# cvlab-yonsei/HVPR

Hardware: AMD Instinct MI355X
Metric: KITTI frames/sec/GPU (fwd, ~20k pts); VFE+scatter achieved HBM GB/s vs peak (higher is better)
Workload: dtype f32; 1 GPU; hvpr_car.yaml batch=1 forward-only, a1..a8 (on-GPU voxelize, pillar VFE, memory read-out + scatter, BEV backbone, head + decode, score top-k + rotated-BEV NMS); frames sharded over ranks, replicas only; global_batch=1, weights=deterministic synthetic (seed 0), BN stats randomised, cls bias -4.595

## Files before the change

### hvpr_amd/_lib.py

```python
import ctypes
import os

_HERE = os.path.dirname(os.path.abspath(__file__))
ABI_VERSION = 7
LIB_PATH = os.environ.get("HVPR_AMD_LIB", os.path.join(_HERE, "libhvpr_amd.so"))

_c = ctypes
_P = _c.c_void_p
_I = _c.c_int
_F = _c.c_float
_Z = _c.c_size_t
ALLREDUCE_FN = _c.CFUNCTYPE(_I, _P, _I, _P, _P)

SIGNATURES = {
    "hvpr_abi_version": (_I, []),
    "hvpr_status_string": (_c.c_char_p, [_I]),
    "hvpr_set_batchnorm_allreduce": (None, [_P, _P]),
    "hvpr_voxelize_workspace_bytes": (_Z, [_I, _I, _I, _I, _I]),
    "hvpr_voxelize_workspace_reset": (_I, [_P, _Z, _I, _I, _I, _I, _I, _P]),
    "hvpr_voxelize_workspace_status": (_I, [_P, _Z, _I, _I, _I, _I, _I, _P]),
    "hvpr_voxelize_f32": (_I, [_P, _I, _I, _I, _I, _P, _I, _F, _F, _F, _F, _F, _F, _I, _I, _I, _I, _I, _I,
                               _P, _P, _P, _P, _I, _P, _Z, _I, _I, _P]),
    "hvpr_pillar_vfe_fwd_f32": (_I, [_P, _P, _P, _I, _I, _P, _F, _F, _F, _F, _F, _F, _P, _P, _P, _P, _P, _P, _P, _P,
                                     _P, _P, _P, _P]),
    "hvpr_memory_bank_packed_floats": (_Z, [_I]),
    "hvpr_memory_bank_pack_f32": (_I, [_P, _I, _P, _P]),
    "hvpr_memory_readout_fwd_f32": (_I, [_P, _I, _P, _P, _P, _I, _I, _P, _P, _P]),
    "hvpr_scatter_workspace_bytes": (_Z, [_I, _I, _I]),
    "hvpr_memory_scatter_fwd_f32": (_I, [_P, _P, _P, _I, _P, _P, _P, _I, _I, _I, _I, _I, _P, _P, _P, _P, _Z, _P]),
    "hvpr_encode_fwd_f32": (_I, [_P, _I, _I, _I, _I, _P, _I, _F, _F, _F, _F, _F, _F, _I, _I, _I, _I, _I, _I, _F, _F, _F,
                                 _P, _P, _P, _P, _P, _P, _P, _P, _P, _P, _I, _I, _P, _P, _P, _P, _I, _P, _P, _P, _P, _P, _P,
                                 _P, _P, _Z, _I, _I, _I, _P]),
    "hvpr_scatter_bev_fwd_f32": (_I, [_P, _I, _P, _I, _P, _I, _P, _I, _P, _I, _I, _I, _P, _P, _P, _Z, _P]),
    "hvpr_spatial_gate_f32": (_I, [_P, _I, _I, _I, _I, _P, _F, _F, _F, _P, _P]),
    "hvpr_head_decode_f32": (_I, [_P, _I, _I, _I, _I, _I, _I, _I, _P, _P, _P, _F, _F, _F, _P, _P, _P, _P, _P]),
    "hvpr_score_topk_workspace_bytes": (_Z, [_I, _I]),
    "hvpr_score_topk_f32": (_I, [_P, _I, _I, _F, _I, _I, _P, _P, _P, _P, _Z, _P]),
    "hvpr_nms_workspace_bytes": (_Z, [_I]),
    "hvpr_nms_bev_f32": (_I, [_P, _I, _P, _P, _I, _F, _I, _I, _P, _P, _P, _Z, _P]),
    "hvpr_gather_predictions_f32": (_I, [_P, _I, _P, _P, _P, _I, _P, _P, _P, _P, _P]),
    "hvpr_boxes_pairwise_f32": (_I, [_P, _I, _P, _I, _I, _P, _P]),
    "hvpr_furthest_point_sample_f32": (_I, [_P, _I, _I, _I, _P, _P]),
    "hvpr_ball_query_f32": (_I, [_P, _P, _I, _I, _I, _F, _I, _P, _P]),
    "hvpr_three_nn_f32": (_I, [_P, _P, _I, _I, _I, _P, _P, _P]),
    "hvpr_group_points_f32": (_I, [_P, _P, _I, _I, _I, _I, _I, _P, _P]),
    "hvpr_group_points_grad_f32": (_I, [_P, _P, _I, _I, _I, _I, _I, _P, _P]),
    "hvpr_three_interpolate_f32": (_I, [_P, _P, _P, _I, _I, _I, _I, _P, _P]),
    "hvpr_three_interpolate_grad_f32": (_I, [_P, _P, _P, _I, _I, _I, _I, _P, _P]),
    "hvpr_group_rows_f32": (_I, [_P, _P, _P, _P, _I, _I, _I, _I, _I, _I, _P, _P]),
    "hvpr_max_samples_f32": (_I, [_P, _c.c_longlong, _I, _I, _P, _P, _P]),
    "hvpr_max_samples_grad_f32": (_I, [_P, _P, _c.c_longlong, _I, _I, _P, _P]),
    "hvpr_fp_rows_f32": (_I, [_P, _P, _P, _P, _I, _I, _I, _I, _I, _I, _P, _P]),
    "hvpr_spatial_gate_train_workspace_bytes": (_Z, [_I, _I, _I]),
    "hvpr_spatial_gate_train_fwd_f32": (_I, [_P, _I, _I, _I, _I, _P, _P, _P, _P, _F, _P, _P, _P, _P, _P, _P, _Z, _P]),
    "hvpr_spatial_gate_train_bwd_f32": (_I, [_P, _P, _P, _P, _P, _P, _P, _P, _I, _I, _I, _I, _P, _P, _P, _P, _P, _P, _Z, _P]),
    "hvpr_conv2d_wgrad_workspace_bytes": (_Z, [_I, _I, _I, _I, _I, _I, _I]),
    "hvpr_conv2d_wgrad_nhwc_f32": (_I, [_P, _I, _I, _I, _I, _P, _I, _I, _I, _P, _P, _Z, _P]),
    "hvpr_bn_workspace_bytes": (_Z, [_c.c_longlong, _I]),
    "hvpr_bn_stats_nhwc_f32": (_I, [_P, _c.c_longlong, _I, _F, _P, _P, _P, _P, _Z, _P]),
    "hvpr_bn_relu_fwd_nhwc_f32": (_I, [_P, _c.c_longlong, _I, _P, _P, _I, _P, _P, _P, _I, _I, _P]),
    "hvpr_bn_relu_bwd_sums_nhwc_f32": (_I, [_P, _I, _I, _P, _c.c_longlong, _I, _P, _P, _P, _P, _I, _P, _P, _P, _P, _Z, _P]),
    "hvpr_bn_relu_bwd_apply_nhwc_f32": (_I, [_P, _I, _I, _P, _c.c_longlong, _I, _P, _P, _P, _P, _I, _P, _P, _P, _P, _P, _c.c_double, _P]),
    "hvpr_memory_train_workspace_bytes": (_Z, [_I]),
    "hvpr_memory_train_fwd_f32": (_I, [_P, _c.c_longlong, _P, _I, _F, _P, _P, _P, _Z, _P]),
    "hvpr_memory_train_bwd_f32": (_I, [_P, _P, _c.c_longlong, _P, _I, _F, _P, _P, _P, _P, _P, _Z, _P]),
    "hvpr_point_pillar_topk_f32": (_I, [_P, _I, _P, _P, _I, _I, _P, _P]),
    "hvpr_scatter_add_rows_f32": (_I, [_P, _P, _c.c_longlong, _I, _I, _P, _P]),
    "hvpr_segment_sum_rows_f32": (_I, [_P, _c.c_longlong, _I, _I, _P, _P, _P, _c.c_longlong, _P, _c.c_longlong, _P]),
    "hvpr_attend_rows_fwd_f32": (_I, [_P, _I, _P, _c.c_longlong, _P, _I, _I, _P, _P, _P]),
    "hvpr_fused_adam_truewd_f32": (_I, [_P, _P, _P, _P, _c.c_longlong, _F, _F, _F, _F, _F, _I, _P, _P]),
    "hvpr_assign_targets_workspace_bytes": (_Z, [_I, _I]),
    "hvpr_assign_targets_f32": (_I, [_P, _I, _P, _I, _I, _I, _I, _F, _F, _I, _I, _I, _c.c_longlong, _P, _P, _P, _P, _P, _Z, _P]),
    "hvpr_rpn_losses_workspace_bytes": (_Z, [_I, _c.c_longlong]),
    "hvpr_rpn_losses_f32": (_I, [_P, _P, _P, _P, _P, _P, _P, _I, _c.c_longlong, _I, _I, _F, _F, _F, _P, _F, _F, _F, _F, _P, _P, _P, _P,
                                 _P, _Z, _P]),
    "hvpr_mse_loss_workspace_bytes": (_Z, []),
    "hvpr_mse_loss_f32": (_I, [_P, _P, _c.c_longlong, _I, _F, _P, _P, _P, _Z, _P]),
    "hvpr_split_bf16_f32": (_I, [_P, _c.c_longlong, _I, _P, _P]),
    "hvpr_unsplit_bf16_f32": (_I, [_P, _c.c_longlong, _I, _P, _P]),
    "hvpr_conv2d_nhwc_bf16x3": (_I, [_P, _I, _I, _I, _I, _P, _P, _I, _I, _I, _I, _P, _P, _I, _P, _I, _I, _I, _I, _I, _P]),
    "hvpr_deconv_nhwc_bf16x3": (_I, [_P, _I, _I, _I, _I, _P, _P, _I, _I, _I, _I, _P, _I, _I, _I, _P]),
    "hvpr_point_flags_f32": (_I, [_P, _I, _I, _I, _P, _F, _P, _P, _I, _I, _P, _P]),
    "hvpr_compact_workspace_bytes": (_Z, [_I]),
    "hvpr_compact_rows_f32": (_I, [_P, _I, _I, _P, _P, _I, _P, _P, _Z, _P]),
    "hvpr_frame_offsets_f32": (_I, [_P, _I, _I, _I, _P, _P]),
    "hvpr_gather_rows_f32": (_I, [_P, _I, _I, _P, _I, _P, _P]),
    "hvpr_pillar_vfe_train_workspace_bytes": (_Z, []),
    "hvpr_pillar_vfe_train_fwd_f32": (_I, [_P, _P, _P, _I, _I, _P, _P, _P, _P, _P, _P, _F, _F, _F, _F, _F, _F, _F, _P, _P, _P, _P, _P, _P, _Z, _P]),
    "hvpr_pillar_vfe_bwd_f32": (_I, [_P, _P, _P, _I, _I, _P, _P, _P, _P, _P, _P, _F, _F, _F, _F, _F, _F, _F, _P, _P, _P, _P, _P, _P, _P, _P, _Z, _P]),
    "hvpr_conv2d_wino_wgrad_workspace_bytes": (_Z, [_I, _I, _I, _I, _I]),
    "hvpr_conv2d_wino_wgrad_nhwc_f32": (_I, [_P, _I, _I, _I, _I, _P, _I, _P, _P, _Z, _P]),
    "hvpr_conv2d_wino_packed_floats": (_Z, [_I, _I]),
    "hvpr_conv2d_wino_pack_f32": (_I, [_P, _P, _I, _I, _I, _P, _P]),
    "hvpr_conv2d_wino_nhwc_f32": (_I, [_P, _I, _I, _I, _I, _P, _P, _I, _I, _P, _P, _I, _P, _I, _I, _I, _P, _P]),
    "hvpr_conv2d_wino_stats_rows": (_I, [_I, _I, _I]),
    "hvpr_conv2d_s2_dgrad_nhwc_f32": (_I, [_P, _I, _I, _I, _I, _P, _P, _I, _I, _I, _I, _P, _I, _I, _P]),
    "hvpr_bn_train_affine_f32": (_I, [_P, _P, _P, _I, _P, _P, _F, _F, _P, _P, _P, _P, _P, _P]),
    "hvpr_bn_finalize_partials_f32": (_I, [_P, _I, _I, _c.c_longlong, _F, _P, _P, _P, _P]),
    "hvpr_conv2d_nhwc_f32": (_I, [_P, _I, _I, _I, _I, _P, _P, _I, _I, _I, _I, _I, _I, _P, _P, _I, _P, _I, _I, _I, _P]),
}

_lib = None


class HvprLibraryError(RuntimeError):
    pass


def lib():
    global _lib
    if _lib is None:
        if not os.path.exists(LIB_PATH):
            raise HvprLibraryError(
                f"{LIB_PATH} is missing: build it with `python -m hvpr_amd.build` (hipcc --offload-arch=gfx950). "
                "hvpr_amd has no CPU fallback.")
        try:
            L = ctypes.CDLL(LIB_PATH)
        except OSError as e:
            raise HvprLibraryError(f"cannot load {LIB_PATH}: {e}") from e
        for name, (res, args) in SIGNATURES.items():
            fn = getattr(L, name)
            fn.restype = res
            fn.argtypes = args
        if L.hvpr_abi_version() != ABI_VERSION:
            raise HvprLibraryError(f"{LIB_PATH} has ABI version {L.hvpr_abi_version()}, these wrappers need {ABI_VERSION}: "
                                   "rebuild it with `python -m hvpr_amd.build`")
        _lib = L
    return _lib


def check(status, what):
    if status != 0:
        msg = lib().hvpr_status_string(int(status))
        raise RuntimeError(f"{what} failed: {msg.decode() if msg else status}")
```

### hvpr_amd/bev_backbone.py

```python
import collections
import contextlib
import os

import torch
import torch.nn as nn

from . import kernels
from .folding import FoldCache, bn_scale_shift


class ConvLayer(nn.Module):

    def __init__(self, in_channels, out_channels, kernel_size, stride=1, padding=0, use_norm=True, activation=False):
        super().__init__()
        self.conv = nn.Conv2d(in_channels, out_channels, kernel_size=kernel_size, stride=stride, padding=padding)
        self.norm = nn.BatchNorm2d(out_channels, eps=1e-3, momentum=0.01) if use_norm else None
        self.relu = nn.ReLU() if activation else None


class SpatialAttention(nn.Module):

    def __init__(self):
        super().__init__()
        self.spatial = ConvLayer(2, 1, 3, stride=1, padding=1, use_norm=True, activation=False)

    def gate_params(self):
        s, t = bn_scale_shift(self.spatial.norm)
        return (self.spatial.conv.weight.detach().float().reshape(18).contiguous(), float(self.spatial.conv.bias.detach()),
                float(s), float(t))


def _conv_bn_relu(cin, cout, stride=1, zero_pad=False):
    if zero_pad:
        return [nn.ZeroPad2d(1), nn.Conv2d(cin, cout, kernel_size=3, stride=stride, padding=0, bias=False),
                nn.BatchNorm2d(cout, eps=1e-3, momentum=0.01), nn.ReLU()]
    return [nn.Conv2d(cin, cout, kernel_size=3, padding=1, bias=False), nn.BatchNorm2d(cout, eps=1e-3, momentum=0.01), nn.ReLU()]


_TILE_CFG = 1
_WINO_PX_GROUPS = 1

_Level = collections.namedtuple("_Level", "index trunk scale gate sfm_steps deconv coff")
_Plan = collections.namedtuple("_Plan", "levels planes")


def _fold_pack(pack, conv, bn, **kw):
    scale, shift = bn_scale_shift(bn)
    return pack(conv.weight, scale, shift, **kw)


def _nhwc(t):
    return t.permute(0, 2, 3, 1).contiguous()


class _Fork:

    __slots__ = ("main", "sides", "used", "held", "y_event", "y_side", "eager")

    def __init__(self, sides):
        self.main, self.sides, self.used = torch.cuda.current_stream(), sides, []
        self.held = []
        self.y_event = self.y_side = None
        self.eager = not torch.cuda.is_current_stream_capturing()

    def branch(self, i, x, out):
        if not self.sides:
            return contextlib.nullcontext()
        side = self.sides[i]
        self.used.append(side)
        side.wait_stream(self.main)
        if self.y_event is not None and self.y_side is not side:
            side.wait_event(self.y_event)
        self.held.append(x)
        if self.eager:
            x.record_stream(side)
            out.record_stream(side)
        return torch.cuda.stream(side)

    def y_ready(self, i, y):
        if self.sides:
            self.y_side = self.sides[i]
            self.y_event = torch.cuda.Event()
            self.y_event.record(self.y_side)
            self.held.append(y)
            if self.eager:
                y.record_stream(self.y_side)
                if i + 1 < len(self.sides):
                    y.record_stream(self.sides[i + 1])

    def join(self):
        for side in dict.fromkeys(self.used):
            self.main.wait_stream(side)
        self.held.clear()


def _trunk(lv, x, out=None):
    for pc in lv.trunk[:-1]:
        x = kernels.conv2d_nhwc(x, pc)
    return kernels.conv2d_nhwc(x, lv.trunk[-1], out=out)


def _branch(lv, x, y, out, fork, y_out=None):
    with fork.branch(lv.index, x, out):
        y = kernels.conv2d_nhwc(y, lv.scale, out=y_out)
        fork.y_ready(lv.index, y)
        gate = kernels.spatial_gate(y, *lv.gate)
        for pc in lv.sfm_steps:
            x = kernels.conv2d_nhwc(x, pc, gate=gate, resid=x)
            fork.held.append(x)
        fork.held.append(gate)
        kernels.conv2d_nhwc(x, lv.deconv, out=out, out_coff=lv.coff)
    return y


class BaseBEVBackbone_Scale(nn.Module):

    def __init__(self, model_cfg, input_channels):
        super().__init__()
        self.model_cfg = model_cfg
        layer_nums, strides, filters = list(model_cfg.LAYER_NUMS), list(model_cfg.LAYER_STRIDES), list(model_cfg.NUM_FILTERS)
        assert len(layer_nums) == len(strides) == len(filters)
        self.sfm_layer_nums = list(model_cfg.SFM_LAYER_NUMS)
        up_strides, up_filters = list(model_cfg.UPSAMPLE_STRIDES), list(model_cfg.NUM_UPSAMPLE_FILTERS)
        assert len(up_strides) == len(up_filters) == len(layer_nums), "HIP path: one deblock per level"
        scale_filters = list(model_cfg.NUM_SCALE_FILTERS)
        assert len(scale_filters) == len(strides)
        cin = [input_channels] + filters[:-1]
        cin_s = [input_channels // 4] + scale_filters[:-1]
        self.layer_strides, self.layer_nums, self.upsample_strides = strides, layer_nums, up_strides
        self.sfmblocks_down, self.sfmblocks_up = nn.ModuleList(), nn.ModuleList()
        self.scale_layers, self.blocks, self.deblocks = nn.ModuleList(), nn.ModuleList(), nn.ModuleList()
        for i in range(len(layer_nums)):
            layers = _conv_bn_relu(cin[i], filters[i], strides[i], zero_pad=True)
            for _ in range(layer_nums[i]):
                layers += _conv_bn_relu(filters[i], filters[i])
            self.blocks.append(nn.Sequential(*layers))
            self.sfmblocks_down.append(nn.Sequential(*_conv_bn_relu(filters[i], filters[i])))
            s = up_strides[i]
            assert s >= 1 and int(s) == s, "HIP path: integer upsample strides (ConvTranspose2d with kernel == stride)"
            self.deblocks.append(nn.Sequential(
                nn.ConvTranspose2d(filters[i], up_filters[i], int(s), stride=int(s), bias=False),
                nn.BatchNorm2d(up_filters[i], eps=1e-3, momentum=0.01), nn.ReLU()))
            self.scale_layers.append(nn.Sequential(*_conv_bn_relu(cin_s[i], scale_filters[i], strides[i], zero_pad=True)))
        self.up_filters = up_filters
        self.num_bev_features = sum(up_filters)
        self.attention = SpatialAttention()
        self._fold = FoldCache()
        self._sides = None
        self.n_streams = int(os.environ.get("HVPR_BEV_STREAMS", "4"))
        self.conv_precision = os.environ.get("HVPR_CONV_PRECISION", model_cfg.get("CONV_PRECISION", "fp32"))
        assert self.conv_precision in self.PRECISIONS

    PRECISIONS = {"fp32": 0, "bf16x3": 2, "bf16x6": 3}

    def set_conv_precision(self, precision):
        assert precision in self.PRECISIONS
        self.conv_precision = precision
        self._fold.invalidate()

    def _streams(self, device):
        n = len(self.blocks)
        if self.n_streams == 1:
            return []
        if self._sides is None or len(self._sides) != n or self._sides[0].device != device:
            own = [torch.cuda.Stream(device=device) for _ in range(n if self.n_streams >= 4 else 1)]
            self._sides = [own[i % len(own)] for i in range(n)]
        return self._sides

    def train(self, mode=True):
        self._fold.invalidate()
        return super().train(mode)

    def _load_from_state_dict(self, *a, **k):
        self._fold.invalidate()
        return super()._load_from_state_dict(*a, **k)

    def _build_plan(self):
        planes = self.PRECISIONS[self.conv_precision]

        def conv_f32(conv, bn, stride=1):
            return _fold_pack(kernels.pack_conv_auto, conv, bn, stride=stride, tile_cfg=_TILE_CFG, px_groups=_WINO_PX_GROUPS)

        def conv_bf3(conv, bn, stride=1):
            return _fold_pack(kernels.pack_conv_bf3, conv, bn, stride=stride, tile_cfg=4, planes=planes)

        conv = conv_bf3 if planes else conv_f32
        gate = self.attention.gate_params()
        levels, coff = [], 0
        for i, blk in enumerate(self.blocks):
            s = self.layer_strides[i]
            trunk = [conv(blk[1], blk[2], stride=s)] + [conv(blk[4 + 3 * k], blk[5 + 3 * k]) for k in range(self.layer_nums[i])]
            sfm = conv(*self.sfmblocks_down[i][:2])
            scale = conv_f32(*self.scale_layers[i][1:3], stride=s)
            de = self.deblocks[i]
            if planes == 2 and de[0].weight.shape[0] % 64 == 0:
                deconv = _fold_pack(kernels.pack_deconv_bf3, de[0], de[1], planes=planes)
            else:
                deconv = _fold_pack(kernels.pack_deconv, de[0], de[1], tile_cfg=_TILE_CFG)
            sfm_steps = [sfm] * self.sfm_layer_nums[i]
            if planes and sfm_steps and isinstance(deconv, kernels.PackedConv):
                sfm_steps[-1] = sfm.fp32_output()
            levels.append(_Level(i, trunk, scale, gate, sfm_steps, deconv, coff))
            coff += self.up_filters[i]
        return _Plan(levels, planes)

    def _forward_train(self, data_dict):
        if not data_dict["spatial_features"].is_cuda:
            raise RuntimeError("hvpr_amd: BaseBEVBackbone_Scale's training forward needs GPU tensors (the HIP path has no CPU fallback)")
        from . import conv_train as ct

        def nhwc(t):
            return t.permute(0, 2, 3, 1).contiguous()

        def cbr(seq, t, gate=None, resid=None):
            mods, k = list(seq), 0
            while k < len(mods):
                if isinstance(mods[k], nn.ZeroPad2d):
                    k += 1
                conv, bn = mods[k], mods[k + 1]
                last = k + 3 >= len(mods)
                if last and gate is not None and resid is t and conv.stride[0] == 1 and conv.kernel_size[0] == 3:
                    t = ct.sfm_step(t, conv.weight, bn, gate)
                else:
                    z, partials = ct.conv(t, conv.weight, conv.stride[0], stats=True)
                    t = ct.bn_relu(z, bn, gate=gate if last else None, resid=resid if last else None, partials=partials)
                k += 3
            return t

        def gate(y, uses):
            sp = self.attention.spatial
            g, mean, var = ct.spatial_gate_train(y, sp.conv.weight, sp.conv.bias, sp.norm.weight, sp.norm.bias, sp.norm.eps)
            ct.update_running_repeated(sp.norm, mean, var, ct.global_count(y.numel() // y.shape[-1], y.device), uses)
            return g

        x, xp = nhwc(data_dict["spatial_features"]), nhwc(data_dict["spatial_features_point"])
        y = nhwc(data_dict["spatial_scale_features"])
        ups, ups_p = [], []
        for i in range(len(self.blocks)):
            x = cbr(self.blocks[i], x)
            xp = cbr(self.blocks[i], xp)
            y = cbr(self.scale_layers[i], y)
            xa, xpa = x, xp
            nsfm = self.sfm_layer_nums[i]
            if nsfm > 0:
                g = gate(y, 2 * nsfm)
                for _ in range(nsfm):
                    xa = cbr(self.sfmblocks_down[i], xa, gate=g, resid=xa)
                    xpa = cbr(self.sfmblocks_down[i], xpa, gate=g, resid=xpa)
            de = self.deblocks[i]
            ups.append(ct.deconv(xa, de[0].weight))
            ups_p.append(ct.deconv(xpa, de[0].weight))
        bns = [de[1] for de in self.deblocks]
        data_dict["spatial_features_2d"] = ct.bn_relu_cat(ups, bns).permute(0, 3, 1, 2)
        data_dict["spatial_features_point_2d"] = ct.bn_relu_cat(ups_p, bns).permute(0, 3, 1, 2)
        return data_dict

    def _head(self, plan, x, y, out, level, x_out={}, y_out=None):
        fork = _Fork(self._streams(y.device))
        for lv in plan.levels:
            x = _trunk(lv, x, out=x_out.get(lv.index))
            if lv.index < level:
                y = _branch(lv, x, y, out, fork, y_out=y_out if lv.index == level - 1 else None)
        fork.join()

    def forward(self, data_dict):
        if self.training:
            return self._forward_train(data_dict)
        x, y = _nhwc(data_dict["spatial_features"]), _nhwc(data_dict["spatial_scale_features"])
        plan = self._fold.get(y.device, self._build_plan)
        B, H, W, _ = x.shape
        s0, us0 = self.layer_strides[0], int(self.upsample_strides[0])
        out = torch.empty((B, ((H + 2 - 3) // s0 + 1) * us0, ((W + 2 - 3) // s0 + 1) * us0, self.num_bev_features),
                          dtype=torch.float32, device=x.device)
        if plan.planes:
            x = kernels.split_bf16(x, plan.planes)
        self._head(plan, x, y, out, len(plan.levels))
        data_dict["spatial_features_2d"] = out.permute(0, 3, 1, 2)
        return data_dict

    def forward_head(self, spatial, scale, split):
        y = _nhwc(scale)
        plan = self._fold.get(y.device, self._build_plan)
        assert not plan.planes, "the split forward runs the fp32 kernels"
        self._head(plan, _nhwc(spatial), y, split["out"], split["level"], split["x"], split["y"])

    def forward_tail(self, split):
        y, out = split["y"], split["out"]
        plan = self._fold.get(y.device, self._build_plan)
        assert not plan.planes, "the split forward runs the fp32 kernels"
        fork = _Fork([])
        for lv in plan.levels[split["level"]:]:
            y = _branch(lv, split["x"][lv.index], y, out, fork)
        fork.join()
        return out.permute(0, 3, 1, 2)

    def split_buffers(self, batch_size, H, W, device, level=None):
        n_lv = len(self.blocks)
        if level is None:
            level = n_lv - 1
        assert 1 <= level <= n_lv - 1
        h, w, hw = H, W, []
        for s in self.layer_strides:
            h, w = (h + 2 - 3) // s + 1, (w + 2 - 3) // s + 1
            hw.append((h, w))
        cy = self.scale_layers[level - 1][1].weight.shape[0]
        us0 = int(self.upsample_strides[0])
        mk = lambda *shape: torch.empty(shape, dtype=torch.float32, device=device)
        return {"level": level,
                "x": {i: mk(batch_size, hw[i][0], hw[i][1], self.blocks[i][1].weight.shape[0]) for i in range(level, n_lv)},
                "y": mk(batch_size, hw[level - 1][0], hw[level - 1][1], cy),
                "out": mk(batch_size, hw[0][0] * us0, hw[0][1] * us0, self.num_bev_features)}


__all__ = {
    "BaseBEVBackbone_Scale": BaseBEVBackbone_Scale,
}
```

### hvpr_amd/csrc/conv_wino.hip

```cpp
#include <type_traits>

#include "common.h"

namespace {

typedef float f32x16 __attribute__((ext_vector_type(16)));
constexpr int KC = 8;
constexpr int BN = 64;
constexpr int TW = 16, PW = TW + 2;
constexpr int ROWP = 20;
constexpr int W_V4 = 16 * 2 * BN;

__device__ __forceinline__ void lds_dma16(const void *sbase_uniform, unsigned voff_bytes, unsigned lds_dst_uniform) {
    unsigned keep;
    asm volatile("s_mov_b32 %0, m0\n\ts_mov_b32 m0, %3\n\ts_nop 0\n\tglobal_load_lds_dwordx4 %1, %2\n\ts_mov_b32 m0, %0"
                 : "=&s"(keep)
                 : "v"(voff_bytes), "s"(sbase_uniform), "s"(lds_dst_uniform)
                 : "memory");
}

__device__ __forceinline__ unsigned lds_addr_of(const void *p) {
    return (unsigned)(size_t)(const __attribute__((address_space(3))) void *)p;
}

struct WinoArgs {
    const float *in;
    const float *wpk;
    const float *bias;
    float *out;
    const float *gate;
    const float *resid;
    int N, H, W, Cin;
    int cout, cout_pad;
    int out_cstride, out_coff, resid_cstride;
    int relu;
    int tiles_x, tiles_y, n_ct;
    float *stats;
};

__device__ __forceinline__ float4 f4_fma(float s, float4 a, float4 b) {
    return make_float4(fmaf(s, a.x, b.x), fmaf(s, a.y, b.y), fmaf(s, a.z, b.z), fmaf(s, a.w, b.w));
}
__device__ __forceinline__ float4 f4_add(float4 a, float4 b) { return make_float4(a.x + b.x, a.y + b.y, a.z + b.z, a.w + b.w); }
__device__ __forceinline__ float4 f4_sub(float4 a, float4 b) { return make_float4(a.x - b.x, a.y - b.y, a.z - b.z, a.w - b.w); }

template <int NG, bool STATS, int NB>
__global__ void __launch_bounds__(256 * NG) __attribute__((amdgpu_waves_per_eu(2, NB == 2 ? 2 : 3))) k_wino(WinoArgs a) {
    constexpr int NT = 256 * NG;
    constexpr int TH = 8 * NG, PH = TH + 2;
    constexpr int PPAD = (PH * ROWP + 63) / 64 * 64;
    constexpr int PATCH_V4 = 2 * PPAD;
    constexpr int BNT = 32 * NB, W_V4T = 16 * 2 * BNT;
    constexpr int NLD_P = (PATCH_V4 + NT - 1) / NT, NLD_W = W_V4T / NT;
    constexpr int PATCH_PAD = NLD_P * NT;
    static_assert(W_V4T % NT == 0 && (NB == 2 || NG == 1), "whole DMA pieces");
    extern __shared__ __attribute__((aligned(16))) float4 smem[];
    float4 *const s_w = smem;
    float4 *const s_patch = smem + 2 * W_V4T;

    const int tid = threadIdx.x, lane = tid & 63, wid = tid >> 6;
    const unsigned wave_s = __builtin_amdgcn_readfirstlane((unsigned)(threadIdx.x >> 6));
    const int grp = wid >> 2, wa = wid & 3;
    const int half = lane >> 5, l31 = lane & 31;
    const int by = l31 >> 3, bx = l31 & 7;

    int p_py[NLD_P], p_px[NLD_P], p_part[NLD_P];
    bool p_live[NLD_P];
#pragma unroll
    for (int i = 0; i < NLD_P; ++i) {
        const int v = tid + i * NT;
        const int plane = v / PPAD, slot = v % PPAD;
        const int y = slot / ROWP, rem = slot % ROWP;
        const int x = 2 * (rem % 10) + rem / 10;
        p_py[i] = y; p_px[i] = x; p_part[i] = plane * 4;
        p_live[i] = plane < 2 && y < PH && x < PW;
    }
    const int r0 = wa == 0 ? 0 : (wa == 2 ? 2 : 1), r1 = wa == 2 ? 1 : (wa == 3 ? 3 : 2);
    const float sgn = wa == 1 ? 1.f : -1.f;
    const int pbase = half * PPAD + (2 * (4 * grp + by)) * ROWP + bx;
    const int p_off0 = pbase + r0 * ROWP, p_off1 = pbase + r1 * ROWP;
    const int u_off = (wa * 4 * 2 + half) * BNT + l31;
    const unsigned lds_w0 = lds_addr_of(s_w) + wave_s * 1024u;
    const unsigned lds_patch0 = lds_addr_of(s_patch) + wave_s * 1024u;

    const int n_pt = a.tiles_x * a.tiles_y * a.N;
    const int total_walk = ((n_pt + 7) / 8) * 8 * a.n_ct;
    const int n_chunks = a.Cin / KC;
    for (int it = blockIdx.x; it < total_walk; it += gridDim.x) {
    const int xcd = it & 7, j = it >> 3;
    const int ct = j % a.n_ct;
    int pt = (j / a.n_ct) * 8 + xcd;
    if (pt >= n_pt) continue;
    const int tx = pt % a.tiles_x; pt /= a.tiles_x;
    const int ty = pt % a.tiles_y;
    const int n = pt / a.tiles_y;
    const int oy0 = ty * TH, ox0 = tx * TW;
    const int iy0 = oy0 - 1, ix0 = ox0 - 1;
    const int co0 = ct * BNT;

    unsigned poff[NLD_P];
    bool pok[NLD_P];
#pragma unroll
    for (int i = 0; i < NLD_P; ++i) {
        const int iy = iy0 + p_py[i], ix = ix0 + p_px[i];
        pok[i] = p_live[i] && iy >= 0 && iy < a.H && ix >= 0 && ix < a.W;
        poff[i] = pok[i] ? (unsigned)(((iy * a.W + ix) * a.Cin + p_part[i]) * (int)sizeof(float)) : 0u;
    }
    const char *in_n = (const char *)(a.in + (size_t)n * a.H * a.W * a.Cin);
    const char *w_ct = (const char *)(a.wpk + (size_t)(NB == 2 ? ct : ct >> 1) * n_chunks * (W_V4 * 4));
    const unsigned w_half = NB == 2 ? 0u : (unsigned)(ct & 1) * 32u * 16u;

    auto stage_piece = [&](int chunk, int buf, int i) {
        if (i < NLD_P) {
            const char *pbase_g = in_n + (size_t)chunk * (KC * sizeof(float));
            if (pok[i]) lds_dma16(pbase_g, poff[i], lds_patch0 + (unsigned)(buf * PATCH_PAD + i * NT) * 16u);
        } else {
            const int j = i - NLD_P;
            const char *wbase = w_ct + (size_t)chunk * (W_V4 * 16);
            lds_dma16(wbase, NB == 2 ? (unsigned)((tid + j * NT) * 16) : (unsigned)((((tid + j * NT) >> 5) * 64 + ((tid + j * NT) & 31)) * 16) + w_half,
                      lds_w0 + (unsigned)(buf * W_V4T + j * NT) * 16u);
        }
    };
    auto stage = [&](int chunk, int buf) {
#pragma unroll
        for (int i = 0; i < NLD_P + NLD_W; ++i) stage_piece(chunk, buf, i);
    };
    const bool border = iy0 < 0 || ix0 < 0 || iy0 + PH > a.H || ix0 + PW > a.W;
    if (border) {
#pragma unroll
        for (int b = 0; b < 2; ++b)
#pragma unroll
            for (int i = 0; i < NLD_P; ++i) s_patch[b * PATCH_PAD + tid + i * NT] = make_float4(0.f, 0.f, 0.f, 0.f);
        __syncthreads();
    }
    static_assert(PH * ROWP + BNT / 4 <= PPAD, "room for the bias row behind the patch");
    if (tid < BNT / 4) s_patch[PH * ROWP + tid] = *(const float4 *)(a.bias + co0 + tid * 4);
    f32x16 acc[4][NB];
#pragma unroll
    for (int b = 0; b < 4; ++b)
#pragma unroll
        for (int nb = 0; nb < NB; ++nb)
#pragma unroll
            for (int r = 0; r < 16; ++r) acc[b][nb][r] = 0.f;

    auto chunk_step = [&](int c, auto buf_tag) {
        constexpr int BUF = decltype(buf_tag)::value;
        asm volatile("s_waitcnt vmcnt(0)" ::: "memory");
        __builtin_amdgcn_s_barrier();
        const float4 *sp = s_patch + BUF * PATCH_PAD;
        const float4 *sw = s_w + BUF * W_V4T;
        float4 d0[4], d1[4], u[4][NB];
#pragma unroll
        for (int jx = 0; jx < 4; ++jx) {
            d0[jx] = sp[p_off0 + (jx & 1) * 10 + (jx >> 1)];
            d1[jx] = sp[p_off1 + (jx & 1) * 10 + (jx >> 1)];
        }
#pragma unroll
        for (int b = 0; b < 2; ++b)
#pragma unroll
            for (int nb = 0; nb < NB; ++nb) u[b][nb] = sw[u_off + b * 2 * BNT + nb * 32];
        __builtin_amdgcn_sched_barrier(0);
        float4 t[4], v[4];
#pragma unroll
        for (int jx = 0; jx < 4; ++jx) t[jx] = f4_fma(sgn, d1[jx], d0[jx]);
        v[0] = f4_sub(t[0], t[2]); v[1] = f4_add(t[1], t[2]); v[2] = f4_sub(t[2], t[1]); v[3] = f4_sub(t[1], t[3]);
#pragma unroll
        for (int b = 0; b < 4; ++b) {
            if (b + 2 < 4) {
#pragma unroll
                for (int nb = 0; nb < NB; ++nb) u[b + 2][nb] = sw[u_off + (b + 2) * 2 * BNT + nb * 32];
            }
            __builtin_amdgcn_sched_barrier(0);
#pragma unroll
            for (int nb = 0; nb < NB; ++nb) {
                acc[b][nb] = __builtin_amdgcn_mfma_f32_32x32x2f32(u[b][nb].x, v[b].x, acc[b][nb], 0, 0, 0);
                acc[b][nb] = __builtin_amdgcn_mfma_f32_32x32x2f32(u[b][nb].y, v[b].y, acc[b][nb], 0, 0, 0);
                acc[b][nb] = __builtin_amdgcn_mfma_f32_32x32x2f32(u[b][nb].z, v[b].z, acc[b][nb], 0, 0, 0);
                acc[b][nb] = __builtin_amdgcn_mfma_f32_32x32x2f32(u[b][nb].w, v[b].w, acc[b][nb], 0, 0, 0);
                constexpr int DEAL = 4 * NB > 5 ? 5 : 4 * NB - 1, NPF = (NLD_P + NLD_W + DEAL - 1) / DEAL;
                static_assert(DEAL * NPF >= NLD_P + NLD_W, "every piece goes out");
                if (c + 1 < n_chunks && b * NB + nb < DEAL) {
                    __builtin_amdgcn_sched_barrier(0);
#pragma unroll
                    for (int i = (b * NB + nb) * NPF; i < (b * NB + nb + 1) * NPF && i < NLD_P + NLD_W; ++i) stage_piece(c + 1, BUF ^ 1, i);
                    __builtin_amdgcn_sched_barrier(0);
                }
            }
            __builtin_amdgcn_sched_barrier(0);
        }
    };
    stage(0, 0);
    for (int c = 0; c + 1 < n_chunks; c += 2) {
        chunk_step(c, std::integral_constant<int, 0>{});
        chunk_step(c + 1, std::integral_constant<int, 1>{});
    }
    if (n_chunks & 1) chunk_step(n_chunks - 1, std::integral_constant<int, 0>{});

    const int p = wa >> 1, q = wa & 1;
    const int oy = oy0 + 2 * (4 * grp + by) + p, ox = ox0 + 2 * bx + q;
    const bool live_px = oy < a.H && ox < a.W;
    const size_t pix = ((size_t)n * a.H + (live_px ? oy : 0)) * a.W + (live_px ? ox : 0);
    const float gate = a.gate && live_px ? a.gate[pix] : 0.f;
    const float *rrow = a.gate ? a.resid + pix * a.resid_cstride : nullptr;
    const float sg = p ? -1.f : 1.f;
    constexpr int NPASS = NG == 1 ? 1 : 2, NBP = NB / NPASS;
    float4 ykeep[2][4];
#pragma unroll
    for (int i = 0; i < 8; ++i) ykeep[i >> 2][i & 3] = make_float4(0.f, 0.f, 0.f, 0.f);
#pragma unroll
    for (int ps = 0; ps < NPASS; ++ps) {
        __syncthreads();
#pragma unroll
        for (int nl = 0; nl < NBP; ++nl) {
            const int nb = ps * NBP + nl;
#pragma unroll
            for (int g = 0; g < 4; ++g) {
                float4 m[4];
#pragma unroll
                for (int b = 0; b < 4; ++b) m[b] = make_float4(acc[b][nb][4 * g], acc[b][nb][4 * g + 1], acc[b][nb][4 * g + 2], acc[b][nb][4 * g + 3]);
                s_w[((((grp * 4 + wa) * 2 + 0) * NBP + nl) * 4 + g) * 64 + lane] = f4_add(f4_add(m[0], m[1]), m[2]);
                s_w[((((grp * 4 + wa) * 2 + 1) * NBP + nl) * 4 + g) * 64 + lane] = f4_sub(f4_sub(m[1], m[2]), m[3]);
            }
        }
        __syncthreads();
        if (live_px) {
#pragma unroll
            for (int nl = 0; nl < NBP; ++nl) {
                const int nb = ps * NBP + nl;
#pragma unroll
                for (int g = 0; g < 4; ++g) {
                    const int col = co0 + nb * 32 + 8 * g + 4 * half;
                    if (col >= a.cout) continue;
                    const float4 x0 = s_w[((((grp * 4 + p) * 2 + q) * NBP + nl) * 4 + g) * 64 + lane];
                    const float4 x1 = s_w[((((grp * 4 + p + 1) * 2 + q) * NBP + nl) * 4 + g) * 64 + lane];
                    const float4 x2 = s_w[((((grp * 4 + p + 2) * 2 + q) * NBP + nl) * 4 + g) * 64 + lane];
                    const float4 bias = s_patch[PH * ROWP + (col - co0) / 4];
                    float4 y = f4_add(f4_fma(sg, x2, f4_fma(sg, x1, x0)), bias);
                    if (a.relu) { y.x = fmaxf(y.x, 0.f); y.y = fmaxf(y.y, 0.f); y.z = fmaxf(y.z, 0.f); y.w = fmaxf(y.w, 0.f); }
                    if (a.gate) {
                        const float4 r = *(const float4 *)(rrow + col);
                        y.x = fmaf(gate, y.x, r.x); y.y = fmaf(gate, y.y, r.y); y.z = fmaf(gate, y.z, r.z); y.w = fmaf(gate, y.w, r.w);
                    }
                    *(float4 *)(a.out + pix * a.out_cstride + a.out_coff + col) = y;
                    if (STATS) ykeep[nl][g] = y;
                }
            }
        }
    }
    static_assert(!STATS || (NG == 1 && NB == 2), "the statistics pass is written for the 8 x 16 px x 64 channel tile");
    if (STATS) {
        __syncthreads();
#pragma unroll
        for (int nl = 0; nl < 2; ++nl)
#pragma unroll
            for (int g = 0; g < 4; ++g) s_w[((wid * 2 + nl) * 4 + g) * 64 + lane] = ykeep[nl][g];
        __syncthreads();
        {
            const int c = tid & 63, part = tid >> 6;
            const float *base = (const float *)(s_w + ((part * 2 + (c >> 5)) * 4 + ((c >> 3) & 3)) * 64 + ((c >> 2) & 1) * 32) + (c & 3);
            float sm = 0.f, sq = 0.f;
#pragma unroll 8
            for (int i = 0; i < 32; ++i) {
                const float v = base[((i + c) & 31) * 4];
                sm += v; sq = fmaf(v, v, sq);
            }
            float *s_part = (float *)(s_w + 2048);
            s_part[(part * 2 + 0) * 64 + c] = sm;
            s_part[(part * 2 + 1) * 64 + c] = sq;
        }
        __syncthreads();
        if (tid < 128) {
            const float *s_part = (const float *)(s_w + 2048);
            const int c = tid & 63, k = tid >> 6;
            const float v = (s_part[(0 * 2 + k) * 64 + c] + s_part[(1 * 2 + k) * 64 + c]) + (s_part[(2 * 2 + k) * 64 + c] + s_part[(3 * 2 + k) * 64 + c]);
            const int pt_lin = (n * a.tiles_y + ty) * a.tiles_x + tx;
            if (co0 + c < a.cout) a.stats[((size_t)pt_lin * 2 + k) * a.cout + co0 + c] = v;
        }
    }
    __syncthreads();
    }
}

__global__ void k_wino_pack(const float *__restrict__ w, const float *__restrict__ scale, int cout, int cin, int cout_pad, int adjoint,
                            float *__restrict__ out) {
    const long long id = blockIdx.x * (long long)blockDim.x + threadIdx.x;
    if (id >= (long long)cout_pad * cin) return;
    const int o = (int)(id / cin), i = (int)(id % cin);
    double g[3][3];
#pragma unroll
    for (int u = 0; u < 3; ++u)
#pragma unroll
        for (int v = 0; v < 3; ++v) {
            double x = 0.0;
            if (o < cout) x = adjoint ? (double)w[(((size_t)i * cout + o) * 3 + (2 - u)) * 3 + (2 - v)] : (double)w[(((size_t)o * cin + i) * 3 + u) * 3 + v];
            g[u][v] = (scale && o < cout) ? x * (double)scale[o] : x;
        }
    double gg[4][3];
#pragma unroll
    for (int v = 0; v < 3; ++v) {
        gg[0][v] = g[0][v];
        gg[1][v] = 0.5 * (g[0][v] + g[1][v] + g[2][v]);
        gg[2][v] = 0.5 * (g[0][v] - g[1][v] + g[2][v]);
        gg[3][v] = g[2][v];
    }
    const int ct = o / BN, co_l = o % BN, chunk = i / KC, hf = (i % KC) / 4, e = i % 4;
    float *dst = out + ((size_t)ct * (cin / KC) + chunk) * (W_V4 * 4);
#pragma unroll
    for (int r = 0; r < 4; ++r) {
        const double U[4] = {gg[r][0], 0.5 * (gg[r][0] + gg[r][1] + gg[r][2]), 0.5 * (gg[r][0] - gg[r][1] + gg[r][2]), gg[r][2]};
#pragma unroll
        for (int b = 0; b < 4; ++b) dst[(((size_t)(r * 4 + b) * 2 + hf) * BN + co_l) * 4 + e] = (float)U[b];
    }
}

template <int NG, bool STATS, int NB>
int launch(WinoArgs a, hipStream_t s) {
    constexpr int NT = 256 * NG, TH = 8 * NG, PH = TH + 2;
    constexpr int PPAD = (PH * ROWP + 63) / 64 * 64;
    constexpr int NLD_P = (2 * PPAD + NT - 1) / NT;
    constexpr int lds = (2 * (16 * 2 * 32 * NB) + 2 * NLD_P * NT) * 16;
    a.tiles_x = (a.W + TW - 1) / TW;
    a.tiles_y = (a.H + TH - 1) / TH;
    a.n_ct = a.cout_pad / (32 * NB);
    static unsigned long long lds_set = 0ull;
    if (hvpr_ensure_dyn_lds((const void *)k_wino<NG, STATS, NB>, lds, &lds_set) != 0) return -1;
    const long long tiles = (long long)a.N * a.tiles_x * a.tiles_y * a.n_ct;
    static int resident = 0;
    if (resident == 0) {
        int per_cu = 0, dev = 0, cus = 256;
        hipDeviceProp_t prop;
        if (hipGetDevice(&dev) == hipSuccess && hipGetDeviceProperties(&prop, dev) == hipSuccess) cus = prop.multiProcessorCount;
        if (hipOccupancyMaxActiveBlocksPerMultiprocessor(&per_cu, k_wino<NG, STATS, NB>, NT, lds) != hipSuccess || per_cu < 1) per_cu = 1;
        resident = per_cu * cus;
    }
    long long blocks = tiles < resident ? (tiles + 7) / 8 * 8 : resident;
    if (blocks > resident && resident >= 8) blocks = resident / 8 * 8;
    hipLaunchKernelGGL((k_wino<NG, STATS, NB>), dim3((unsigned)blocks), dim3(NT), lds, s, a);
    return 0;
}

}

extern "C" int hvpr_conv2d_wino_stats_rows(int N, int H, int W) {
    if (N < 1 || H < 1 || W < 1) return 0;
    return N * ((H + 7) / 8) * ((W + TW - 1) / TW);
}

extern "C" size_t hvpr_conv2d_wino_packed_floats(int cin, int cout) {
    if (cin < 1 || cout < 1) return 0;
    return (size_t)((cout + BN - 1) / BN * BN) * (size_t)cin * 16;
}

extern "C" int hvpr_conv2d_wino_pack_f32(const float *weight, const float *scale, int cout, int cin, int adjoint, float *packed,
                                         hvpr_stream_t stream) {
    if (!weight || !packed || cout < 1 || cin < 1) return HVPR_ERR_INVALID_ARG;
    if (cin % KC != 0) return HVPR_ERR_UNSUPPORTED;
    const int cout_pad = (cout + BN - 1) / BN * BN;
    const long long n = (long long)cout_pad * cin;
    hipLaunchKernelGGL(k_wino_pack, dim3(hvpr_cdiv(n, 256)), dim3(256), 0, (hipStream_t)stream, weight, scale, cout, cin, cout_pad,
                       adjoint ? 1 : 0, packed);
    HVPR_CHECK_LAUNCH();
    return HVPR_OK;
}

extern "C" int hvpr_conv2d_wino_nhwc_f32(const float *in, int N, int H, int W, int Cin, const float *w_packed, const float *bias,
                                         int cout, int relu, const float *gate, const float *resid, int resid_cstride, float *out,
                                         int out_cstride, int out_coff, int px_groups, float *bn_partials, hvpr_stream_t stream) {
    if (!in || !w_packed || !bias || !out || N < 1 || H < 1 || W < 1 || Cin < 8 || cout < 1) return HVPR_ERR_INVALID_ARG;
    if ((gate == nullptr) != (resid == nullptr)) return HVPR_ERR_INVALID_ARG;
    if (Cin % KC != 0) return HVPR_ERR_UNSUPPORTED;
    if (cout % 4 != 0 || out_cstride % 4 != 0 || out_coff % 4 != 0 || (resid && resid_cstride % 4 != 0)) return HVPR_ERR_UNSUPPORTED;
    if ((long long)H * W * Cin * 4 >= (1ll << 31)) return HVPR_ERR_UNSUPPORTED;
    WinoArgs a;
    a.in = in; a.wpk = w_packed; a.bias = bias; a.out = out; a.gate = gate; a.resid = resid;
    a.N = N; a.H = H; a.W = W; a.Cin = Cin;
    a.cout = cout; a.cout_pad = (cout + BN - 1) / BN * BN;
    a.out_cstride = out_cstride; a.out_coff = out_coff; a.resid_cstride = resid_cstride;
    a.relu = relu;
    a.stats = bn_partials;
    if (bn_partials && (px_groups != 1 || relu || gate)) return HVPR_ERR_UNSUPPORTED;
    int rc;
    if (px_groups == 1) rc = bn_partials ? launch<1, true, 2>(a, (hipStream_t)stream) : launch<1, false, 2>(a, (hipStream_t)stream);
    else if (px_groups == 2) rc = launch<2, false, 2>(a, (hipStream_t)stream);
    else if (px_groups == 4) rc = launch<1, false, 1>(a, (hipStream_t)stream);
    else return HVPR_ERR_INVALID_ARG;
    if (rc != 0) return HVPR_ERR_LAUNCH;
    HVPR_CHECK_LAUNCH();
    return HVPR_OK;
}
```

### hvpr_amd/csrc/internal.h

```cpp
#pragma once
#include "common.h"

#define HVPR_INTERNAL __attribute__((visibility("hidden")))

constexpr int kScanThreads = 256;
constexpr int kScanItems = 2;
constexpr int kScanTile = kScanThreads * kScanItems;
constexpr int kIdle = 0x7fffffff;

struct VoxWs {
    int *cell_first;
    int *cell_count;
    int *cell_vid;
    int *pt_cell;
    int4 *vox_rec;
    int *arena;
    float4 *arena_pt;
    int4 *arena_rec;
    int *arena_total;
    float *vfe_aux;
    int *frame_base;
    unsigned long long *tile_state;
    int *ticket;
    unsigned long long *cell_pack;
    int *sync;
};

static inline VoxWs hvpr_vox_carve(void *ws, int batch, int n, long long ncell, size_t *bytes = nullptr) {
    hvpr_carver c(ws);
    VoxWs w;
    w.cell_first = c.take<int>((size_t)batch * ncell);
    w.cell_count = c.take<int>((size_t)batch * ncell);
    w.cell_vid = c.take<int>((size_t)batch * ncell);
    w.pt_cell = c.take<int>(n);
    w.vox_rec = c.take<int4>(n);
    w.arena = c.take<int>(n);
    w.arena_pt = c.take<float4>(n);
    w.arena_rec = c.take<int4>(n);
    w.arena_total = c.take<int>(1);
    w.vfe_aux = c.take<float>(128);
    w.frame_base = c.take<int>(batch + 1);
    w.tile_state = c.take<unsigned long long>(hvpr_cdiv(n > 0 ? n : 1, kScanTile));
    w.ticket = c.take<int>(1);
    w.cell_pack = c.take<unsigned long long>((size_t)batch * ncell);
    w.sync = c.take<int>(8 + 64);
    if (bytes) *bytes = c.off;
    return w;
}

static inline size_t hvpr_vox_ws_bytes(int batch, int n, long long ncell) {
    size_t bytes = 0;
    hvpr_vox_carve(nullptr, batch, n, ncell, &bytes);
    return bytes;
}

struct ClearJob {
    int *cell_first;
    int *cell_count;
    const int *cell_vid;
    const int *frame_base;
    const int *voxel_offsets;
    int batch, nx, ny, max_voxels, capacity;
    float *spatial;
    float *spatial_scale;
    long long cell_lo, cell_hi;
    unsigned char *state;
};

__device__ __forceinline__ void hvpr_canvas_clear(const ClearJob &c, int blk, int nblk) {
    constexpr int V = 32, VS = 8;
    typedef float f32x4 __attribute__((ext_vector_type(4)));
    const int lane = threadIdx.x & 63;
    const long long wave = ((long long)blk * blockDim.x + threadIdx.x) >> 6, n_waves = ((long long)nblk * blockDim.x) >> 6;
    const f32x4 zero = {0.f, 0.f, 0.f, 0.f};
    for (long long c0 = c.cell_lo + wave * 64; c0 < c.cell_hi; c0 += n_waves * 64) {
        const long long cell = c0 + lane;
        bool emitted = false, stale = c.state == nullptr;
        if (cell < c.cell_hi) {
            if (c.state) stale = c.state[cell] != 0;
            if (c.cell_first[cell] != kIdle) {
                c.cell_first[cell] = kIdle;
                c.cell_count[cell] = 0;
                const int b = (int)(cell / ((long long)c.nx * c.ny));
                const int local = c.cell_vid[cell] - c.frame_base[b];
                emitted = local < c.max_voxels && c.voxel_offsets[b] + local < c.capacity;
            }
            if (c.state && stale != emitted) c.state[cell] = emitted ? 1 : 0;
        }
        const unsigned long long skip = __ballot(emitted || !stale);
        if (c.state && skip == ~0ull) continue;
        f32x4 *const main = reinterpret_cast<f32x4 *>(c.spatial) + c0 * V;
        f32x4 *const side = reinterpret_cast<f32x4 *>(c.spatial_scale) + c0 * VS;
        const int cells = (int)min(64ll, c.cell_hi - c0);
#pragma unroll 8
        for (int i = lane; i < cells * V; i += 64)
            if (!((skip >> (i / V)) & 1ull)) __builtin_nontemporal_store(zero, main + i);
#pragma unroll 8
        for (int i = lane; i < cells * VS; i += 64)
            if (!((skip >> (i / VS)) & 1ull)) __builtin_nontemporal_store(zero, side + i);
    }
}

typedef float hvpr_f32x16 __attribute__((ext_vector_type(16)));
__device__ __forceinline__ void hvpr_vfe_padded_slot(const float (&aw)[2][8], const float (&b0h)[8], float *z1) {
    const int lane = threadIdx.x & 63, h = lane >> 5, slot = lane & 31;
#pragma unroll
    for (int mb = 0; mb < 2; ++mb) {
        hvpr_f32x16 acc = {0.f, 0.f, 0.f, 0.f, 0.f, 0.f, 0.f, 0.f, 0.f, 0.f, 0.f, 0.f, 0.f, 0.f, 0.f, 0.f};
#pragma unroll
        for (int t = 0; t < 8; ++t) acc = __builtin_amdgcn_mfma_f32_32x32x2f32(aw[mb][t], fmaxf(0.f + b0h[t], 0.f), acc, 0, 0, 0);
        if (slot == 0) {
#pragma unroll
            for (int g = 0; g < 4; ++g) *(float4 *)&z1[32 * mb + 8 * g + 4 * h] = make_float4(acc[4 * g], acc[4 * g + 1], acc[4 * g + 2], acc[4 * g + 3]);
        }
    }
}

struct VoxelizeArgs {
    const float *points;
    int n_points, point_stride, xyz_col, n_feat;
    const int32_t *frame_offsets;
    int batch;
    float lo_x, lo_y, lo_z, vs_x, vs_y, vs_z;
    int nx, ny, nz, max_points, max_voxels, cap_mode;
};

struct VfeWeights {
    float vs_x, vs_y, vs_z, off_x, off_y, off_z;
    const float *w0, *b0, *w1, *b1, *ws0, *bs0, *ws1, *bs1;
};

struct WarmSmall { const float *p[8]; int n[8]; };
HVPR_INTERNAL int hvpr_i_voxel_index(const VoxelizeArgs &a, const VoxWs &w, int32_t *voxel_offsets, bool for_encode,
                                     hipStream_t s, const float *vfe_w1 = nullptr, const float *vfe_b0 = nullptr,
                                     const void *warm0 = nullptr, size_t warm0_bytes = 0, const void *warm1 = nullptr, size_t warm1_bytes = 0,
                                     const WarmSmall *warm_small = nullptr, int index_mode = 0);
HVPR_INTERNAL int hvpr_i_vfe_gather(const VoxelizeArgs &a, const VoxWs &w, const int32_t *voxel_offsets, int capacity,
                                    const VfeWeights &v, float *voxels, int32_t *coords, int32_t *num_points,
                                    float *pillar_features, float *scale_features, float *pillar_mask, float *spatial,
                                    int spatial_channels, float *spatial_scale, unsigned char *canvas_state, hipStream_t s);
HVPR_INTERNAL int hvpr_i_readout(const float *f, int M, const int32_t *m_device, const float *bank, const float *bank_packed, int n_items, int k,
                                 float *out, int32_t *topk_idx, const int32_t *coords, int batch, int nx, int ny,
                                 int *cell_map, float *canvas, int canvas_channels, int canvas_offset, hipStream_t s);
```

### hvpr_amd/detector.py

```python
import os

import numpy as np
import torch
import torch.nn as nn

from . import anchor_head, bev_backbone, iou3d_nms_utils, kernels, map_to_bev, pointnet2, vfe
from .voxel_generator import VoxelGenerator

backbones_3d_all = pointnet2.__all__
REGISTRY = {
    "backbone_3d": backbones_3d_all,
    "vfe": vfe.__all__,
    "map_to_bev": map_to_bev.__all__,
    "backbone_2d": bev_backbone.__all__,
    "dense_head": anchor_head.__all__,
}


def class_agnostic_nms(box_scores, box_preds, nms_config, score_thresh=None):
    n = box_scores.shape[0]
    dev = box_scores.device
    if n == 0:
        return torch.zeros((0,), dtype=torch.long, device=dev), box_scores[:0]
    pre = min(int(nms_config.NMS_PRE_MAXSIZE), n)
    ws = kernels.PostWorkspace(1, n, pre, dev)
    order, _, cnt = kernels.score_topk(box_scores.float().reshape(1, n).contiguous(), score_thresh, pre, ws, want_scores=False)
    keep, kc = kernels.nms_bev(box_preds.float().contiguous(), order[0].contiguous(), cnt, pre, float(nms_config.NMS_THRESH),
                               int(nms_config.NMS_POST_MAXSIZE), ws.nms)
    selected = keep[: int(kc.item())].long()
    return selected, box_scores[selected]


def multi_classes_nms(cls_scores, box_preds, nms_config, score_thresh=None):
    pred_scores, pred_labels, pred_boxes = [], [], []
    for k in range(cls_scores.shape[1]):
        col = cls_scores[:, k].contiguous()
        selected, sc = class_agnostic_nms(col, box_preds, nms_config, score_thresh=score_thresh)
        pred_scores.append(sc)
        pred_labels.append(torch.full((selected.shape[0],), k, dtype=torch.long, device=col.device))
        pred_boxes.append(box_preds[selected])
    return torch.cat(pred_scores, dim=0), torch.cat(pred_labels, dim=0), torch.cat(pred_boxes, dim=0)


class Detector3DTemplate(nn.Module):

    def __init__(self, model_cfg, num_class, dataset):
        super().__init__()
        self.model_cfg = model_cfg
        self.num_class = num_class
        self.dataset = dataset
        self.class_names = dataset.class_names
        self.register_buffer("global_step", torch.LongTensor(1).zero_())
        self.module_topology = ["backbone_3d", "vfe", "map_to_bev_module", "pfe", "backbone_2d", "dense_head",
                                "point_head", "roi_head"]
        self._post_ws = None

    @property
    def mode(self):
        return "TRAIN" if self.training else "TEST"

    def update_global_step(self):
        self.global_step += 1

    def build_networks(self):
        info = {
            "module_list": [],
            "num_rawpoint_features": self.dataset.point_feature_encoder.num_point_features,
            "num_point_features": self.dataset.point_feature_encoder.num_point_features,
            "grid_size": self.dataset.grid_size,
            "point_cloud_range": self.dataset.point_cloud_range,
            "voxel_size": self.dataset.voxel_size,
        }
        for name in self.module_topology:
            module, info = getattr(self, "build_%s" % name)(model_info_dict=info)
            self.add_module(name, module)
        return info["module_list"]

    def build_backbone_3d(self, model_info_dict):
        cfg = self.model_cfg.get("BACKBONE_3D", None)
        if cfg is None or cfg.NAME not in backbones_3d_all:
            return None, model_info_dict
        m = backbones_3d_all[cfg.NAME](model_cfg=cfg, input_channels=model_info_dict["num_point_features"],
                                       grid_size=model_info_dict["grid_size"], voxel_size=model_info_dict["voxel_size"],
                                       point_cloud_range=model_info_dict["point_cloud_range"])
        model_info_dict["module_list"].append(m)
        model_info_dict["num_point_features"] = m.num_point_features
        return m, model_info_dict

    def build_vfe(self, model_info_dict):
        cfg = self.model_cfg.get("VFE", None)
        if cfg is None:
            return None, model_info_dict
        m = vfe.__all__[cfg.NAME](model_cfg=cfg, num_point_features=model_info_dict["num_rawpoint_features"],
                                  point_cloud_range=model_info_dict["point_cloud_range"], voxel_size=model_info_dict["voxel_size"])
        model_info_dict["num_point_features"] = m.get_output_feature_dim()
        model_info_dict["module_list"].append(m)
        return m, model_info_dict

    def build_map_to_bev_module(self, model_info_dict):
        cfg = self.model_cfg.get("MAP_TO_BEV", None)
        if cfg is None:
            return None, model_info_dict
        m = map_to_bev.__all__[cfg.NAME](model_cfg=cfg, grid_size=model_info_dict["grid_size"])
        model_info_dict["module_list"].append(m)
        model_info_dict["num_bev_features"] = m.num_bev_features
        return m, model_info_dict

    def build_backbone_2d(self, model_info_dict):
        cfg = self.model_cfg.get("BACKBONE_2D", None)
        if cfg is None:
            return None, model_info_dict
        m = bev_backbone.__all__[cfg.NAME](model_cfg=cfg, input_channels=model_info_dict["num_bev_features"])
        model_info_dict["module_list"].append(m)
        model_info_dict["num_bev_features"] = m.num_bev_features
        return m, model_info_dict

    def build_dense_head(self, model_info_dict):
        cfg = self.model_cfg.get("DENSE_HEAD", None)
        if cfg is None:
            return None, model_info_dict
        m = anchor_head.__all__[cfg.NAME](
            model_cfg=cfg, input_channels=model_info_dict["num_bev_features"],
            num_class=self.num_class if not cfg.CLASS_AGNOSTIC else 1, class_names=self.class_names,
            grid_size=model_info_dict["grid_size"], point_cloud_range=model_info_dict["point_cloud_range"],
            predict_boxes_when_training=self.model_cfg.get("ROI_HEAD", False))
        model_info_dict["module_list"].append(m)
        return m, model_info_dict

    def _absent(self, key, model_info_dict):
        assert self.model_cfg.get(key, None) is None, f"{key} is outside the hvpr hot path"
        return None, model_info_dict

    def build_pfe(self, model_info_dict):
        return self._absent("PFE", model_info_dict)

    def build_point_head(self, model_info_dict):
        return self._absent("POINT_HEAD", model_info_dict)

    def build_roi_head(self, model_info_dict):
        return self._absent("ROI_HEAD", model_info_dict)

    def forward(self, **kwargs):
        raise NotImplementedError

    def post_processing(self, batch_dict, sync=True):
        cfg = self.model_cfg.POST_PROCESSING
        ncfg = cfg.NMS_CONFIG
        if ncfg.MULTI_CLASSES_NMS:
            return self._post_processing_multi_class(batch_dict)
        B = batch_dict["batch_size"]
        boxes_all = batch_dict["batch_box_preds"]
        assert boxes_all.dim() == 3 and boxes_all.shape[0] == B
        cls_all = batch_dict["batch_cls_preds"]
        assert cls_all.shape[2] in (1, self.num_class)
        if "batch_max_scores" in batch_dict:
            scores, labels = batch_dict["batch_max_scores"], batch_dict["batch_max_labels"]
        else:
            c = cls_all if batch_dict["cls_preds_normalized"] else torch.sigmoid(cls_all)
            scores, lab = torch.max(c, dim=-1)
            labels = (lab + 1).to(torch.int32)
        A = scores.shape[1]
        pre, post = min(int(ncfg.NMS_PRE_MAXSIZE), A), int(ncfg.NMS_POST_MAXSIZE)
        dev = scores.device
        if self._post_ws is None or (self._post_ws.batch, self._post_ws.n_scores, self._post_ws.pre_max) != (B, A, pre) \
                or self._post_ws.topk.device != dev:
            self._post_ws = kernels.PostWorkspace(B, A, pre, dev)
        order, _, counts = kernels.score_topk(scores.contiguous(), cfg.SCORE_THRESH, pre, self._post_ws, want_scores=False)
        pred_dicts, recall_dict = [], {}
        for b in range(B):
            keep, kc = kernels.nms_bev(boxes_all[b], order[b], counts[b:b + 1], pre, float(ncfg.NMS_THRESH), post,
                                       self._post_ws.nms)
            if labels.dtype == torch.int32 and not cfg.OUTPUT_RAW_SCORE and boxes_all[b].is_contiguous():
                pb, ps, pl, sel = kernels.gather_predictions(boxes_all[b], scores[b].contiguous(), labels[b].contiguous(), keep)
                rec = {"pred_boxes": pb, "pred_labels": pl, "pred_scores": ps, "selected": sel, "pred_count": kc}
            else:
                sel = keep.long()
                rec = {"pred_boxes": boxes_all[b].index_select(0, sel), "pred_labels": labels[b].index_select(0, sel).long(),
                       "pred_scores": (cls_all[b].max(dim=-1)[0] if cfg.OUTPUT_RAW_SCORE else scores[b]).index_select(0, sel),
                       "selected": sel, "pred_count": kc}
            if sync:
                n = int(kc.item())
                rec = {k: (v[:n] if k != "pred_count" else v) for k, v in rec.items()}
                recall_dict = self.generate_recall_record(rec["pred_boxes"], recall_dict, b, batch_dict, cfg.RECALL_THRESH_LIST)
            pred_dicts.append(rec)
        return pred_dicts, recall_dict, batch_dict

    def _post_processing_multi_class(self, batch_dict):
        cfg = self.model_cfg.POST_PROCESSING
        pred_dicts, recall_dict = [], {}
        for b in range(batch_dict["batch_size"]):
            cls = batch_dict["batch_cls_preds"][b]
            cls = cls if batch_dict["cls_preds_normalized"] else torch.sigmoid(cls)
            boxes = batch_dict["batch_box_preds"][b]
            mapping = torch.arange(1, cls.shape[1] + 1, device=cls.device)
            sc, lab, bx = multi_classes_nms(cls.float(), boxes, cfg.NMS_CONFIG, score_thresh=cfg.SCORE_THRESH)
            rec = {"pred_boxes": bx, "pred_scores": sc, "pred_labels": mapping[lab]}
            recall_dict = self.generate_recall_record(bx, recall_dict, b, batch_dict, cfg.RECALL_THRESH_LIST)
            pred_dicts.append(rec)
        return pred_dicts, recall_dict, batch_dict

    @staticmethod
    def generate_recall_record(box_preds, recall_dict, batch_index, data_dict=None, thresh_list=None):
        if "gt_boxes" not in data_dict:
            return recall_dict
        gt = data_dict["gt_boxes"][batch_index]
        if len(recall_dict) == 0:
            recall_dict = {"gt": 0}
            for t in thresh_list:
                recall_dict["roi_%s" % str(t)] = 0
                recall_dict["rcnn_%s" % str(t)] = 0
        row_is_zero = (gt.sum(dim=1) == 0).tolist()
        k = len(row_is_zero) - 1
        while k > 0 and row_is_zero[k]:
            k -= 1
        gt = gt[:k + 1]
        if gt.shape[0] > 0:
            if box_preds.shape[0] > 0:
                best = iou3d_nms_utils.boxes_iou3d_gpu(box_preds[:, 0:7], gt[:, 0:7]).max(dim=0)[0]
                thr = torch.tensor([float(t) for t in thresh_list], dtype=best.dtype).to(best.device, non_blocking=True)
                recalled = (best.unsqueeze(0) > thr.unsqueeze(1)).sum(dim=1).tolist()
                for t, n in zip(thresh_list, recalled):
                    recall_dict["rcnn_%s" % str(t)] += int(n)
            recall_dict["gt"] += gt.shape[0]
        return recall_dict

    def load_params_from_file(self, filename, logger=None, to_cpu=False):
        ckpt = torch.load(filename, map_location=torch.device("cpu") if to_cpu else None)
        disk = ckpt["model_state"]
        state = self.state_dict()
        update = {k: v for k, v in disk.items() if k in state and state[k].shape == v.shape}
        state.update(update)
        self.load_state_dict(state)
        from . import conv_train
        conv_train.weights_changed()
        if logger is not None:
            for k in state:
                if k not in update:
                    logger.info("Not updated weight %s: %s" % (k, str(state[k].shape)))
            logger.info("==> Done (loaded %d/%d)" % (len(update), len(state)))
        return len(update), len(state)


    def load_params_with_optimizer(self, filename, to_cpu=False, optimizer=None, logger=None):
        if not os.path.isfile(filename):
            raise FileNotFoundError(filename)
        ckpt = torch.load(filename, map_location=torch.device("cpu") if to_cpu else None)
        self.load_state_dict(ckpt["model_state"])
        if optimizer is not None:
            ost = ckpt.get("optimizer_state")
            if ost is None:
                stem, ext = os.path.splitext(filename)
                side = "%s_optim%s" % (stem, ext)
                if os.path.exists(side):
                    ost = torch.load(side, map_location=torch.device("cpu") if to_cpu else None)["optimizer_state"]
            if ost is not None:
                optimizer.load_state_dict(ost)
        if logger is not None:
            logger.info("==> Resumed from %s (epoch %s, it %s, version %s)" % (filename, ckpt.get("epoch", -1), ckpt.get("it", 0.0),
                                                                              ckpt.get("version", "none")))
        return ckpt.get("it", 0.0), ckpt.get("epoch", -1)


class _VoxelizingDetector(Detector3DTemplate):

    def __init__(self, model_cfg, num_class, dataset):
        super().__init__(model_cfg=model_cfg, num_class=num_class, dataset=dataset)
        self._voxgen = {}

    def _voxel_cfg(self):
        for p in self.dataset.dataset_cfg.DATA_PROCESSOR:
            if p.NAME == "transform_points_to_voxels":
                return p
        raise KeyError("transform_points_to_voxels")

    def _voxel_generator(self, device):
        mode = "train" if self.training else "test"
        key = (mode, torch.device(device))
        if key not in self._voxgen:
            vc = self._voxel_cfg()
            self._voxgen[key] = VoxelGenerator(vc.VOXEL_SIZE, self.dataset.point_cloud_range, vc.MAX_POINTS_PER_VOXEL,
                                               vc.MAX_NUMBER_OF_VOXELS[mode], device=device)
        return self._voxgen[key]

    @staticmethod
    def _frame_offsets(batch_dict):
        offs = batch_dict.get("point_frame_offsets")
        if offs is None:
            pts, B = batch_dict["points"], batch_dict["batch_size"]
            if pts.is_cuda and pts.dtype == torch.float32 and pts.is_contiguous():
                offs = kernels.frame_offsets(pts, B)
            else:
                offs = torch.searchsorted(pts[:, 0].contiguous(), torch.arange(B + 1, device=pts.device, dtype=pts.dtype)).to(torch.int32)
        return offs

    def voxelize_on_device(self, batch_dict):
        pts = batch_dict["points"]
        B = batch_dict["batch_size"]
        offs = self._frame_offsets(batch_dict)
        v, c, n, vo = self._voxel_generator(pts.device).generate_batch(pts, offs, B, xyz_col=1, n_feat=pts.shape[1] - 1)
        batch_dict["voxels"], batch_dict["voxel_coords"], batch_dict["voxel_num_points"] = v, c, n
        batch_dict["voxel_offsets"] = vo
        batch_dict["voxel_count_device"] = vo[B:B + 1]
        return batch_dict


class MixAnchor_Memory(_VoxelizingDetector):

    def __init__(self, model_cfg, num_class, dataset):
        super().__init__(model_cfg=model_cfg, num_class=num_class, dataset=dataset)
        self.module_list = self.build_networks()
        self.export_voxels = bool(model_cfg.get("EXPORT_VOXELS", False))
        self.index_mode = int(model_cfg.get("ENCODE_INDEX_MODE", 1))

    def get_training_loss(self):
        rpn, rpn_point, mem, tb_dict, items = self.dense_head.get_loss()
        loss = rpn + rpn_point + mem
        tb_dict = {"loss_rpn": rpn.detach(), **tb_dict}
        return loss, tb_dict, {"items": items}

    def _can_fuse_encode(self, batch_dict):
        if self.training or "voxels" in batch_dict:
            return False
        v, m = getattr(self, "vfe", None), getattr(self, "map_to_bev_module", None)
        if not isinstance(v, vfe.PillarVFE_Scale) or not isinstance(m, map_to_bev.PointPillarScatter_Agg_Memory_1_scale):
            return False
        pts = batch_dict["points"]
        return (pts.is_cuda and pts.dim() == 2 and pts.shape[1] == 5 and v.num_filters == [32, 64] and
                v.num_scale_features == [16, 32] and tuple(m.memory.weight.shape[1:]) == (64,) and m.nz == 1 and
                int(self._voxel_cfg().MAX_POINTS_PER_VOXEL) <= 32 and m.memory.weight.shape[0] <= 2048 and m.k <= 32)

    def encode_fused(self, batch_dict):
        pts, B = batch_dict["points"].contiguous(), batch_dict["batch_size"]
        vg = self._voxel_generator(pts.device)
        m = self.map_to_bev_module
        r = kernels.encode_fwd(pts, self._frame_offsets(batch_dict), B, vg.point_cloud_range, vg.voxel_size, vg.grid_size,
                               vg.max_num_points, vg.max_voxels, vg._workspace(B, pts.shape[0]),
                               self.vfe._fold.get(pts.device, self.vfe._build_folded), self.vfe.offsets,
                               m.memory.packed_bank(), m.k, xyz_col=1, cap_mode=vg.cap_mode, want_voxels=self.export_voxels,
                               want_mask=self.export_voxels, out=batch_dict.get("_out_spatial"), state=batch_dict.get("_canvas_state"),
                               index_mode=self.index_mode)
        vo = r["voxel_offsets"]
        batch_dict.update(voxels=r["voxels"], voxel_coords=r["coords"], voxel_num_points=r["num_points"], voxel_offsets=vo,
                          voxel_count_device=vo[B:B + 1], pillar_features=r["pillar_features"],
                          pillar_scale_features=r["pillar_scale_features"], pillar_mask=r["pillar_mask"],
                          spatial_features=r["spatial"], spatial_scale_features=r["spatial_scale"])
        return batch_dict

    def persistent_canvases(self, example_batch):
        if not self._can_fuse_encode(example_batch):
            return {}
        m = self.map_to_bev_module
        canv, state = kernels.canvas_buffers(example_batch["batch_size"], m.nx, m.ny, example_batch["points"].device)
        return {"_out_spatial": canv, "_canvas_state": state}

    def stage_encode(self, batch_dict):
        if self._can_fuse_encode(batch_dict):
            return self.encode_fused(batch_dict)
        if "voxels" not in batch_dict:
            batch_dict = self.voxelize_on_device(batch_dict)
        return self.map_to_bev_module(self.vfe(batch_dict))

    def stage_dense(self, batch_dict):
        return self.dense_head(self.backbone_2d(batch_dict))

    def stage_dense_a(self, batch_dict, split):
        self.backbone_2d.forward_head(batch_dict["spatial_features"], batch_dict["spatial_scale_features"], split)

    def stage_dense_b(self, batch_dict, split):
        return self.dense_head({**batch_dict, "spatial_features_2d": self.backbone_2d.forward_tail(split)})

    def prefetch_point_indices(self, batch_dict):
        pn = getattr(self, "backbone_3d", None)
        if pn is None or not hasattr(pn, "index_plan") or "points" not in batch_dict or not batch_dict["points"].is_cuda:
            return batch_dict
        if getattr(self, "_pn2_stream", None) is None:
            self._pn2_stream = torch.cuda.Stream()
        s = self._pn2_stream
        s.wait_stream(torch.cuda.current_stream())
        with torch.cuda.stream(s):
            plan = pn.index_plan(batch_dict["points"], batch_dict["batch_size"])
            ready = torch.cuda.Event()
            ready.record(s)
        batch_dict["points"].record_stream(s)
        batch_dict["_pn2_plan"] = (plan, ready)
        return batch_dict

    def forward(self, batch_dict, sync=True):
        fused = self._can_fuse_encode(batch_dict)
        if fused:
            batch_dict = self.encode_fused(batch_dict)
        elif "voxels" not in batch_dict:
            batch_dict = self.voxelize_on_device(batch_dict)
        if self.training:
            for m in self.module_list:
                batch_dict = m(batch_dict)
            loss, tb_dict, disp_dict = self.get_training_loss()
            return {"loss": loss}, tb_dict, disp_dict
        for m in self.module_list:
            if m is getattr(self, "backbone_3d", None) or (fused and (m is self.vfe or m is self.map_to_bev_module)):
                continue
            batch_dict = m(batch_dict)
        out = self.post_processing(batch_dict, sync=sync)
        if fused and sync and self.index_mode == 1:
            self._voxel_generator(batch_dict["points"].device)._ws.status()
        return out


class _CapturedState:

    def __init__(self, model):
        self.slots = []
        for m in model.modules():
            if hasattr(m, "_fold") and hasattr(m._fold, "value"):
                self.slots.append((m._fold, "value"))
            if hasattr(m, "_packed"):
                self.slots.append((m, "_packed"))
        self.slots.append((model, "_post_ws"))
        for vg in getattr(model, "_voxgen", {}).values():
            self.slots.append((vg, "_ws"))
        self.keep = [getattr(o, a) for o, a in self.slots]

    def check(self):
        for (o, a), was in zip(self.slots, self.keep):
            if getattr(o, a) is not was:
                raise RuntimeError(f"hvpr_amd: {type(o).__name__}.{a} was rebuilt after this hipGraph was captured (train()/eval(), "
                                   "load_state_dict, set_conv_precision or a workspace re-allocation): capture a new graph")


def _check_voxelizer_status(model):
    for vg in getattr(model, "_voxgen", {}).values():
        if vg._ws is not None:
            vg._ws.status()


class GraphedForward:

    def __init__(self, model, example_batch, warmup=3):
        assert not model.training
        self.model = model
        self.static_in = {k: (v.clone() if torch.is_tensor(v) else v) for k, v in example_batch.items()}
        if hasattr(model, "persistent_canvases"):
            self.static_in.update(model.persistent_canvases(example_batch))
        side = torch.cuda.Stream()
        side.wait_stream(torch.cuda.current_stream())
        with torch.cuda.stream(side), torch.no_grad():
            for _ in range(warmup):
                model(dict(self.static_in), sync=False)
        torch.cuda.current_stream().wait_stream(side)
        torch.cuda.synchronize()
        self.graph = torch.cuda.CUDAGraph()
        with torch.cuda.graph(self.graph), torch.no_grad():
            self.static_out = model(dict(self.static_in), sync=False)
        self.captured = _CapturedState(model)

    def __call__(self, batch):
        self.captured.check()
        for k, v in batch.items():
            if torch.is_tensor(v):
                self.static_in[k].copy_(v, non_blocking=True)
        self.graph.replay()
        return self.static_out

    def check_status(self):
        _check_voxelizer_status(self.model)


class PipelinedForward:

    _HEAD_KEYS = ("batch_cls_preds", "batch_box_preds", "batch_max_scores", "batch_max_labels")

    def __init__(self, model, example_batch, warmup=2, depth=None):
        assert not model.training and hasattr(model, "stage_encode")
        if depth is None:
            fp32 = getattr(model.backbone_2d, "conv_precision", "fp32") == "fp32" and hasattr(model.backbone_2d, "split_buffers")
            depth = 4 if fp32 else 3
        assert depth in (3, 4)
        self.model, self.step, self.depth = model, 0, depth
        self.B = example_batch["batch_size"]
        self.inp = [{k: (v.clone() if torch.is_tensor(v) else v) for k, v in example_batch.items()} for _ in range(2)]
        self.canvas, self.head, self.aux, self.split = [None, None], [None, None], [None, None], [None, None]
        self.enc, self.f2d = [None, None], [None, None]
        self.own = [model.persistent_canvases(example_batch) if hasattr(model, "persistent_canvases") else {} for _ in range(2)]
        side = torch.cuda.Stream()
        side.wait_stream(torch.cuda.current_stream())
        with torch.cuda.stream(side), torch.no_grad():
            for p in range(2):
                for _ in range(warmup):
                    bd = model.stage_encode({**self.inp[p], **self.own[p]})
                    self.canvas[p] = (bd["spatial_features"], bd["spatial_scale_features"])
                    if depth == 4:
                        if self.split[p] is None:
                            sp = bd["spatial_features"]
                            self.split[p] = model.backbone_2d.split_buffers(self.B, sp.shape[2], sp.shape[3], sp.device)
                        model.stage_dense_a(bd, self.split[p])
                        bd = model.stage_dense_b(bd, self.split[p])
                    else:
                        bd = model.stage_dense(bd)
                    self.head[p] = tuple(bd[k] for k in self._HEAD_KEYS)
                    model.post_processing(bd, sync=False)
        torch.cuda.current_stream().wait_stream(side)
        torch.cuda.synchronize()
        self.s_enc, self.s_post, self.s_b = torch.cuda.Stream(), torch.cuda.Stream(), torch.cuda.Stream()
        self.graphs, self.out = [torch.cuda.CUDAGraph(), torch.cuda.CUDAGraph()], [None, None]
        pool = None
        for p in range(2):
            q = 1 - p
            post_lane = p if depth == 3 else q
            with torch.cuda.graph(self.graphs[p], pool=pool), torch.no_grad():
                main = torch.cuda.current_stream()
                self.s_enc.wait_stream(main)
                self.s_post.wait_stream(main)
                with torch.cuda.stream(self.s_post):
                    self.out[p] = model.post_processing(self._post_dict(post_lane), sync=False)[0]
                with torch.cuda.stream(self.s_enc):
                    bd = model.stage_encode({**self.inp[p], "_out_spatial": self.canvas[p], **self.own[p]})
                    self.aux[p] = bd["voxel_offsets"]
                    self.enc[p] = {k: bd[k] for k in ("voxel_coords", "voxel_num_points", "voxel_offsets", "pillar_features",
                                                      "pillar_scale_features") if bd.get(k) is not None}
                dense_in = {"batch_size": self.B, "spatial_features": self.canvas[q][0], "spatial_scale_features": self.canvas[q][1]}
                if depth == 3:
                    self.f2d[q] = model.stage_dense({**dense_in, "_out_head": self.head[q]})["spatial_features_2d"]
                else:
                    self.s_b.wait_stream(main)
                    with torch.cuda.stream(self.s_b):
                        model.stage_dense_b({"batch_size": self.B, "_out_head": self.head[p]}, self.split[p])
                    model.stage_dense_a(dense_in, self.split[q])
                    main.wait_stream(self.s_b)
                main.wait_stream(self.s_enc)
                main.wait_stream(self.s_post)
            pool = self.graphs[p].pool()
        self.captured = _CapturedState(model)

    def _post_dict(self, p):
        d = dict(zip(self._HEAD_KEYS, self.head[p]))
        d.update(batch_size=self.B, cls_preds_normalized=False)
        return d

    def __call__(self, batch):
        self.captured.check()
        p = self.step & 1
        for k, v in batch.items():
            if torch.is_tensor(v):
                self.inp[p][k].copy_(v, non_blocking=True)
        self.graphs[p].replay()
        self.step += 1
        return self.out[p] if self.step >= self.depth else None

    def inspect(self, batch):
        for _ in range(self.depth):
            out = self(batch)
        torch.cuda.synchronize()
        self.check_status()
        p = (self.step - 1) & 1
        q = 1 - p
        d = {k: v.clone() for k, v in self.enc[p].items()}
        d["spatial_features"], d["spatial_scale_features"] = self.canvas[p][0].clone(), self.canvas[p][1].clone()
        if self.depth == 4:
            d["spatial_features_2d"] = self.split[p]["out"].permute(0, 3, 1, 2).clone()
            head_now, head_post = self.head[p], self.head[q]
        else:
            d["spatial_features_2d"] = self.f2d[q].clone()
            head_now, head_post = self.head[q], self.head[p]
        d.update({k: v.clone() for k, v in zip(self._HEAD_KEYS, head_now)})
        d["post_input"] = {k: v.clone() for k, v in zip(self._HEAD_KEYS, head_post)}
        d["post"] = [{k: (v.clone() if torch.is_tensor(v) else v) for k, v in rec.items()} for rec in out]
        return d

    def check_status(self):
        _check_voxelizer_status(self.model)

    def flush(self):
        for _ in range(self.depth - 1):
            p = self.step & 1
            self.graphs[p].replay()
            self.step += 1
            if self.step >= self.depth:
                yield self.out[p]


class PointPillar(_VoxelizingDetector):

    def __init__(self, model_cfg, num_class, dataset):
        super().__init__(model_cfg=model_cfg, num_class=num_class, dataset=dataset)
        self.module_list = self.build_networks()

    def forward(self, batch_dict, sync=True):
        if self.training:
            raise NotImplementedError("hvpr_amd: plain PointPillar has no training path (the reference's own detectors/pointpillar.py:24-32 unpacks "
                                      "two values from a get_loss that returns five, anchor_head_template.py:291); train MixAnchor_Memory")
        if "voxels" not in batch_dict:
            batch_dict = self.voxelize_on_device(batch_dict)
        for m in self.module_list:
            batch_dict = m(batch_dict)
        return self.post_processing(batch_dict, sync=sync)


__all__ = {
    "Detector3DTemplate": Detector3DTemplate,
    "PointPillar": PointPillar,
    "MixAnchor_Memory": MixAnchor_Memory,
}


def build_detector(model_cfg, num_class, dataset):
    return __all__[model_cfg.NAME](model_cfg=model_cfg, num_class=num_class, dataset=dataset)


def build_network(model_cfg, num_class, dataset):
    return build_detector(model_cfg=model_cfg, num_class=num_class, dataset=dataset)


def load_data_to_gpu(batch_dict):
    for k, v in batch_dict.items():
        if not isinstance(v, np.ndarray) or k in ("frame_id", "metadata", "calib", "image_shape"):
            continue
        batch_dict[k] = torch.from_numpy(v).float().cuda()


class SyntheticDataset:

    class _Encoder:
        def __init__(self, n):
            self.num_point_features = n

    def __init__(self, cfg, training=False):
        from .voxel_generator import grid_size_of
        self.dataset_cfg = cfg.DATA_CONFIG
        self.class_names = list(cfg.CLASS_NAMES)
        self.training = training
        self.point_cloud_range = np.array(self.dataset_cfg.POINT_CLOUD_RANGE, dtype=np.float32)
        self.point_feature_encoder = self._Encoder(len(self.dataset_cfg.POINT_FEATURE_ENCODING.used_feature_list))
        vc = [p for p in self.dataset_cfg.DATA_PROCESSOR if p.NAME == "transform_points_to_voxels"][0]
        self.voxel_size = vc.VOXEL_SIZE
        self.grid_size = grid_size_of(self.point_cloud_range, self.voxel_size)
```

### hvpr_amd/kernels.py

```python
import os

import torch

from ._lib import check, lib


def _stream():
    return torch.cuda.current_stream().cuda_stream


def _ptr(t, dtype=None, name="tensor"):
    if t is None:
        return None
    if not t.is_cuda:
        raise RuntimeError(f"hvpr_amd: {name} must live on the GPU (the HIP path has no CPU fallback)")
    if dtype is not None and t.dtype != dtype:
        raise TypeError(f"hvpr_amd: {name} must be {dtype}, got {t.dtype}")
    if not t.is_contiguous():
        raise ValueError(f"hvpr_amd: {name} must be contiguous")
    return t.data_ptr()


class VoxelizeWorkspace:

    def __init__(self, batch, n_points, grid, device):
        self.key = (int(batch), int(n_points), tuple(int(g) for g in grid), torch.device(device))
        nx, ny, nz = self.key[2]
        nbytes = lib().hvpr_voxelize_workspace_bytes(batch, n_points, nx, ny, nz)
        self.buf = torch.empty(nbytes, dtype=torch.uint8, device=device)
        self.reset()

    def reset(self):
        batch, n_points, (nx, ny, nz), _ = self.key
        check(lib().hvpr_voxelize_workspace_reset(self.buf.data_ptr(), self.buf.numel(), batch, n_points, nx, ny, nz,
                                                  _stream()), "hvpr_voxelize_workspace_reset")

    def status(self):
        batch, n_points, (nx, ny, nz), _ = self.key
        check(lib().hvpr_voxelize_workspace_status(self.buf.data_ptr(), self.buf.numel(), batch, n_points, nx, ny, nz,
                                                   _stream()), "hvpr_voxelize_workspace_status")


def voxelize(points, frame_offsets, batch, point_cloud_range, voxel_size, grid, max_points, max_voxels, workspace,
             xyz_col=0, n_feat=None, cap_mode=0, capacity=None):
    n, stride = points.shape
    n_feat = stride - xyz_col if n_feat is None else n_feat
    if capacity is None:
        capacity = min(n, batch * max_voxels)
    dev = points.device
    voxels = torch.empty((capacity, max_points, n_feat), dtype=torch.float32, device=dev)
    coords = torch.empty((capacity, 4), dtype=torch.int32, device=dev)
    num = torch.empty((capacity,), dtype=torch.int32, device=dev)
    offs = torch.empty((batch + 1,), dtype=torch.int32, device=dev)
    nx, ny, nz = [int(g) for g in grid]
    lo = [float(torch.tensor(v, dtype=torch.float32)) for v in point_cloud_range[:3]]
    vs = [float(torch.tensor(v, dtype=torch.float32)) for v in voxel_size]
    if workspace.key[0] < batch or workspace.key[1] < n:
        raise ValueError("voxelize workspace too small for this call")
    check(lib().hvpr_voxelize_f32(_ptr(points, torch.float32, "points"), n, stride, xyz_col, n_feat,
                                  _ptr(frame_offsets, torch.int32, "frame_offsets"), batch, lo[0], lo[1], lo[2],
                                  vs[0], vs[1], vs[2], nx, ny, nz, int(max_points), int(max_voxels), int(cap_mode),
                                  voxels.data_ptr(), coords.data_ptr(), num.data_ptr(), offs.data_ptr(), capacity,
                                  workspace.buf.data_ptr(), workspace.buf.numel(), workspace.key[0], workspace.key[1],
                                  _stream()), "hvpr_voxelize_f32")
    return voxels, coords, num, offs


def pillar_vfe_fwd(voxels, num_points, coords, folded, voxel_size, offsets, m_device=None, want_mask=True):
    M, P, C = voxels.shape
    if C != 4:
        raise ValueError("hvpr_pillar_vfe_fwd_f32 is built for 4 raw point features")
    dev = voxels.device
    pf = torch.empty((M, 64), dtype=torch.float32, device=dev)
    sf = torch.empty((M, 32), dtype=torch.float32, device=dev)
    mask = torch.empty((M, P, 1), dtype=torch.float32, device=dev) if want_mask else None
    check(lib().hvpr_pillar_vfe_fwd_f32(
        _ptr(voxels, torch.float32, "voxels"), _ptr(num_points, torch.int32, "voxel_num_points"),
        _ptr(coords, torch.int32, "voxel_coords"), M, P, _ptr(m_device, torch.int32, "m_device"),
        float(voxel_size[0]), float(voxel_size[1]), float(voxel_size[2]), float(offsets[0]), float(offsets[1]),
        float(offsets[2]), _ptr(folded["w0"], torch.float32), _ptr(folded["b0"], torch.float32),
        _ptr(folded["w1"], torch.float32), _ptr(folded["b1"], torch.float32), _ptr(folded["ws0"], torch.float32),
        _ptr(folded["bs0"], torch.float32), _ptr(folded["ws1"], torch.float32), _ptr(folded["bs1"], torch.float32),
        pf.data_ptr(), sf.data_ptr(), _ptr(mask), _stream()), "hvpr_pillar_vfe_fwd_f32")
    return pf, sf, mask


class PackedBank:

    def __init__(self, weight):
        w = weight.detach().float().contiguous()
        if w.dim() != 2 or w.shape[1] != 64:
            raise ValueError("PackedBank: (n_items, 64) memory bank expected")
        self.n_items = int(w.shape[0])
        self.shape = w.shape
        self.rows = w
        self.data = torch.empty(lib().hvpr_memory_bank_packed_floats(self.n_items), dtype=torch.float32, device=w.device)
        check(lib().hvpr_memory_bank_pack_f32(_ptr(w, torch.float32, "memory.weight"), self.n_items, self.data.data_ptr(), _stream()),
              "hvpr_memory_bank_pack_f32")


def _bank_args(bank):
    if not isinstance(bank, PackedBank):
        _ptr(bank, torch.float32, "memory.weight")
        bank = PackedBank(bank)
    return bank.rows.data_ptr(), bank.data.data_ptr(), bank.n_items


def memory_readout_fwd(f, bank, k, m_device=None, want_idx=False):
    M, C = f.shape
    out = torch.empty((M, C), dtype=torch.float32, device=f.device)
    idx = torch.empty((M, k), dtype=torch.int32, device=f.device) if want_idx else None
    check(lib().hvpr_memory_readout_fwd_f32(_ptr(f, torch.float32, "pillar_features"), M,
                                            _ptr(m_device, torch.int32, "m_device"), *_bank_args(bank), int(k),
                                            out.data_ptr(), _ptr(idx), _stream()), "hvpr_memory_readout_fwd_f32")
    return (out, idx) if want_idx else out


_SEG_CHUNK = 32


def edges_by_destination(dst, n_dst):
    dst = dst.reshape(-1).to(torch.int64)
    dev = dst.device
    E = dst.numel()
    n_max = E // _SEG_CHUNK + min(n_dst, E) + 1
    if E == 0:
        z = torch.zeros(1, dtype=torch.int32, device=dev)
        return torch.zeros(0, dtype=torch.int32, device=dev), z.expand(n_max + 1).contiguous(), z.expand(n_dst + 1).contiguous()
    order = torch.argsort(dst, stable=True)
    sdst = dst[order].contiguous()
    rowptr = torch.searchsorted(sdst, torch.arange(n_dst + 1, dtype=torch.int64, device=dev))
    end_live = rowptr[n_dst:]
    pos = torch.arange(E, dtype=torch.int64, device=dev)
    live = (sdst >= 0) & (sdst < n_dst)
    first = rowptr[sdst.clamp(0, n_dst - 1)]
    head = live & (((pos - first) % _SEG_CHUNK) == 0)
    csum = torch.cumsum(head.to(torch.int64), 0)
    cid, total = csum - 1, csum[-1:]
    chunk_ptr = end_live.expand(n_max + 1).clone()
    chunk_ptr.scatter_(0, torch.where(head, cid, torch.full_like(cid, n_max)), torch.where(head, pos, end_live.expand(E)))
    dest_ptr = torch.where(rowptr < end_live, cid[rowptr.clamp(max=E - 1)], total.expand(n_dst + 1))
    return order.to(torch.int32), chunk_ptr.to(torch.int32), dest_ptr.to(torch.int32)


def segment_sum_rows(src, src_off, C, edge_row, edge_w, chunk_ptr, dest_ptr, n_dst):
    n_chunks = chunk_ptr.numel() - 1
    part = torch.empty((n_chunks, C), dtype=torch.float32, device=src.device)
    check(lib().hvpr_segment_sum_rows_f32(_ptr(src, torch.float32, "src"), src.shape[-1], int(src_off), int(C), _ptr(edge_row, torch.int32, "edge_row"),
                                          _ptr(edge_w, torch.float32, "edge_w"), _ptr(chunk_ptr, torch.int32, "chunk_ptr"), int(n_chunks),
                                          part.data_ptr(), int(C), _stream()), "hvpr_segment_sum_rows_f32")
    dst = torch.empty((n_dst, C), dtype=torch.float32, device=src.device)
    check(lib().hvpr_segment_sum_rows_f32(part.data_ptr(), int(C), 0, int(C), None, None, _ptr(dest_ptr, torch.int32, "dest_ptr"), int(n_dst),
                                          dst.data_ptr(), int(C), _stream()), "hvpr_segment_sum_rows_f32")
    return dst


def attend_rows(q, rows, idx=None, k=None):
    if idx is not None:
        if idx.dim() != 2 or (k is not None and int(k) != idx.shape[1]):
            raise ValueError("hvpr_amd: attend_rows needs idx of shape (M, k)")
        k = idx.shape[1]
    elif k is None:
        raise ValueError("hvpr_amd: attend_rows without idx needs k")
    M, C = q.shape
    if rows.dim() != 2 or rows.shape[1] != C or (idx is not None and idx.shape[0] != M):
        raise ValueError("hvpr_amd: attend_rows needs q (M, C), rows (N, C) and idx (M, k)")
    qp, rp, ip = _ptr(q, torch.float32, "q"), _ptr(rows, torch.float32, "rows"), _ptr(idx, torch.int32, "idx")
    out = torch.empty((M, C), dtype=torch.float32, device=q.device)
    w = torch.empty((M, int(k)), dtype=torch.float32, device=q.device)
    check(lib().hvpr_attend_rows_fwd_f32(qp, M, rp, rows.shape[0], ip, int(k), C, out.data_ptr(), w.data_ptr(), _stream()),
          "hvpr_attend_rows_fwd_f32")
    return out, w


def scatter_workspace(batch, nx, ny, device):
    n = lib().hvpr_scatter_workspace_bytes(batch, nx, ny) // 4
    return torch.full((n,), -1, dtype=torch.int32, device=device)


def scatter_bev_fwd(pillar, memory, scale, coords, batch, nx, ny, workspace, m_device=None):
    M, cp = pillar.shape
    cm = 0 if memory is None else memory.shape[1]
    cs = 0 if scale is None else scale.shape[1]
    dev = pillar.device
    spatial = torch.empty((batch, ny, nx, cp + cm), dtype=torch.float32, device=dev)
    spatial_scale = torch.empty((batch, ny, nx, cs), dtype=torch.float32, device=dev) if cs else None
    check(lib().hvpr_scatter_bev_fwd_f32(_ptr(pillar, torch.float32, "pillar_features"), cp, _ptr(memory, torch.float32),
                                         cm, _ptr(scale, torch.float32), cs, _ptr(coords, torch.int32, "voxel_coords"),
                                         M, _ptr(m_device, torch.int32), batch, nx, ny, spatial.data_ptr(),
                                         _ptr(spatial_scale), workspace.data_ptr(), workspace.numel() * 4, _stream()),
          "hvpr_scatter_bev_fwd_f32")
    spatial = spatial.permute(0, 3, 1, 2)
    if spatial_scale is not None:
        spatial_scale = spatial_scale.permute(0, 3, 1, 2)
    return spatial, spatial_scale


class PackedConvBf3:

    def __init__(self, w, bias, cin, cout, cout_pad, stride, relu, tile_cfg, planes, up=None, out_split=True):
        self.w, self.bias, self.cin, self.cout, self.cout_pad = w, bias, cin, cout, cout_pad
        self.stride, self.relu, self.tile_cfg, self.planes, self.up, self.out_split = stride, relu, tile_cfg, planes, up, out_split

    def fp32_output(self):
        return PackedConvBf3(self.w, self.bias, self.cin, self.cout, self.cout_pad, self.stride, self.relu, self.tile_cfg, self.planes,
                             out_split=False)


def _planes_of(x, planes):
    out, r = [], x
    for _ in range(planes):
        h = r.to(torch.bfloat16)
        out.append(h)
        r = r - h.float()
    return out


def pack_conv_bf3(weight, scale=None, shift=None, stride=1, relu=True, tile_cfg=0, planes=2):
    cout, cin, kh, kw = weight.shape
    assert kh == kw == 3 and cin % 16 == 0 and cout % 4 == 0 and planes in (2, 3)
    w = weight.detach().float()
    if scale is not None:
        w = w * scale.view(-1, 1, 1, 1)
    cout_pad = (cout + 63) // 64 * 64
    wp = torch.zeros((9, cin // 8, planes, cout_pad, 8), dtype=torch.bfloat16, device=w.device)
    for k, part in enumerate(_planes_of(w, planes)):
        wp[:, :, k, :cout, :] = part.permute(2, 3, 1, 0).reshape(9, cin // 8, 8, cout).permute(0, 1, 3, 2)
    b = torch.zeros((cout_pad,), dtype=torch.float32, device=w.device)
    if shift is not None:
        b[:cout] = shift.detach().float()
    return PackedConvBf3(wp.contiguous(), b, cin, cout, cout_pad, stride, relu, tile_cfg, planes)


def pack_deconv_bf3(weight, scale, shift, relu=True, planes=2):
    cin, cout, s, s2 = weight.shape
    assert s == s2 and cin % 64 == 0 and cout % 4 == 0 and planes in (2, 3)
    w = weight.detach().float() * scale.view(1, -1, 1, 1)
    cols = s * s * cout
    cout_pad = (cols + 63) // 64 * 64
    g = w.permute(0, 2, 3, 1).reshape(cin, cols)
    wp = torch.zeros((1, cin // 8, planes, cout_pad, 8), dtype=torch.bfloat16, device=w.device)
    for k, part in enumerate(_planes_of(g, planes)):
        wp[0, :, k, :cols, :] = part.reshape(cin // 8, 8, cols).permute(0, 2, 1)
    b = torch.zeros((cout_pad,), dtype=torch.float32, device=w.device)
    b[:cols] = shift.detach().float().repeat(s * s)
    return PackedConvBf3(wp.contiguous(), b, cin, cout, cout_pad, 1, relu, 1, planes, up=s)


def deconv_nhwc_bf3(xs, pc, out, out_coff=0):
    N, H, W, groups, planes, _ = xs.shape
    assert groups * 8 == pc.cin and planes == pc.planes and xs.is_contiguous()
    assert out.shape[:3] == (N, H * pc.up, W * pc.up) and out.is_contiguous() and out.dtype == torch.float32
    check(lib().hvpr_deconv_nhwc_bf16x3(xs.data_ptr(), N, H, W, pc.cin, pc.w.data_ptr(), pc.bias.data_ptr(), pc.cout, pc.cout_pad,
                                        pc.up, 1 if pc.relu else 0, out.data_ptr(), out.shape[-1], out_coff, planes, _stream()),
          "hvpr_deconv_nhwc_bf16x3")
    return out


def split_bf16(x, planes=2):
    assert x.is_contiguous() and x.shape[-1] % 8 == 0 and x.dtype == torch.float32
    out = torch.empty((*x.shape[:-1], x.shape[-1] // 8, planes, 8), dtype=torch.bfloat16, device=x.device)
    check(lib().hvpr_split_bf16_f32(_ptr(x, torch.float32, "activations"), x.numel(), planes, out.data_ptr(), _stream()),
          "hvpr_split_bf16_f32")
    return out


def unsplit_bf16(xs):
    assert xs.is_contiguous() and xs.dtype == torch.bfloat16 and xs.shape[-1] == 8
    planes = xs.shape[-2]
    out = torch.empty((*xs.shape[:-3], xs.shape[-3] * 8), dtype=torch.float32, device=xs.device)
    check(lib().hvpr_unsplit_bf16_f32(xs.data_ptr(), out.numel(), planes, out.data_ptr(), _stream()), "hvpr_unsplit_bf16_f32")
    return out


def conv2d_nhwc_bf3(xs, pc, out_split=True, gate=None, resid=None):
    N, H, W, groups, planes, _ = xs.shape
    cin = groups * 8
    assert cin == pc.cin and planes == pc.planes and xs.is_contiguous()
    OH, OW = (H + 2 - 3) // pc.stride + 1, (W + 2 - 3) // pc.stride + 1
    if out_split:
        assert pc.cout % 8 == 0
        out = torch.empty((N, OH, OW, pc.cout // 8, planes, 8), dtype=torch.bfloat16, device=xs.device)
    else:
        out = torch.empty((N, OH, OW, pc.cout), dtype=torch.float32, device=xs.device)
    check(lib().hvpr_conv2d_nhwc_bf16x3(xs.data_ptr(), N, H, W, cin, pc.w.data_ptr(), pc.bias.data_ptr(), pc.stride, pc.cout,
                                        pc.cout_pad, 1 if pc.relu else 0, _ptr(gate, torch.float32, "gate"),
                                        None if resid is None else resid.data_ptr(), 0 if resid is None else resid.shape[3] * 8,
                                        out.data_ptr(), 1 if out_split else 0, pc.cout, 0, pc.tile_cfg, planes, _stream()),
          "hvpr_conv2d_nhwc_bf16x3")
    return out


def memory_scatter_fwd(pillar, scale, coords, bank, k, batch, nx, ny, workspace, m_device=None, out=None):
    M = pillar.shape[0]
    dev = pillar.device
    mem = torch.empty((M, 64), dtype=torch.float32, device=dev)
    if out is not None:
        spatial, spatial_scale = (o.permute(0, 2, 3, 1) for o in out)
        if spatial.shape != (batch, ny, nx, 128) or spatial_scale.shape != (batch, ny, nx, 32) or not spatial.is_contiguous() \
                or not spatial_scale.is_contiguous():
            raise ValueError("memory_scatter_fwd: `out` canvases do not match this call")
    else:
        spatial = torch.empty((batch, ny, nx, 128), dtype=torch.float32, device=dev)
        spatial_scale = torch.empty((batch, ny, nx, 32), dtype=torch.float32, device=dev)
    if pillar.shape[1] != 64 or scale.shape[1] != 32 or bank.shape[1] != 64:
        raise ValueError("memory_scatter_fwd is specialised for 64 pillar / 64 memory / 32 scale channels")
    check(lib().hvpr_memory_scatter_fwd_f32(_ptr(pillar, torch.float32, "pillar_features"), _ptr(scale, torch.float32, "scale"),
                                            _ptr(coords, torch.int32, "voxel_coords"), M, _ptr(m_device, torch.int32),
                                            *_bank_args(bank), int(k), batch, nx, ny,
                                            mem.data_ptr(), spatial.data_ptr(), spatial_scale.data_ptr(), workspace.data_ptr(),
                                            workspace.numel() * 4, _stream()), "hvpr_memory_scatter_fwd_f32")
    return mem, spatial.permute(0, 3, 1, 2), spatial_scale.permute(0, 3, 1, 2)


def frame_offsets(points, batch):
    offs = torch.empty((batch + 1,), dtype=torch.int32, device=points.device)
    check(lib().hvpr_frame_offsets_f32(_ptr(points, torch.float32, "points"), points.shape[0], points.shape[1], int(batch),
                                       offs.data_ptr(), _stream()), "hvpr_frame_offsets_f32")
    return offs


def encode_fwd(points, frame_offsets, batch, point_cloud_range, voxel_size, grid, max_points, max_voxels, workspace, folded,
               offsets, bank, k, xyz_col=0, cap_mode=0, capacity=None, want_voxels=True, want_mask=True, out=None, state=None,
               index_mode=0):
    n, stride = points.shape
    n_feat = stride - xyz_col
    if capacity is None:
        capacity = min(n, batch * max_voxels)
    dev = points.device
    nx, ny, nz = [int(g) for g in grid]
    voxels = torch.empty((capacity, max_points, n_feat), dtype=torch.float32, device=dev) if want_voxels else None
    coords = torch.empty((capacity, 4), dtype=torch.int32, device=dev)
    num = torch.empty((capacity,), dtype=torch.int32, device=dev)
    offs = torch.empty((batch + 1,), dtype=torch.int32, device=dev)
    pf = torch.empty((capacity, 64), dtype=torch.float32, device=dev)
    sf = torch.empty((capacity, 32), dtype=torch.float32, device=dev)
    mem = torch.empty((capacity, 64), dtype=torch.float32, device=dev)
    mask = torch.empty((capacity, max_points, 1), dtype=torch.float32, device=dev) if want_mask else None
    if out is not None:
        spatial, spatial_scale = (o.permute(0, 2, 3, 1) for o in out)
        if spatial.shape != (batch, ny, nx, 128) or spatial_scale.shape != (batch, ny, nx, 32) or not spatial.is_contiguous() \
                or not spatial_scale.is_contiguous():
            raise ValueError("encode_fwd: `out` canvases do not match this call")
    else:
        spatial = torch.empty((batch, ny, nx, 128), dtype=torch.float32, device=dev)
        spatial_scale = torch.empty((batch, ny, nx, 32), dtype=torch.float32, device=dev)
    if bank.shape[1] != 64:
        raise ValueError("encode_fwd is specialised for 64 pillar / 64 memory / 32 scale channels")
    if state is not None and (out is None or state.dtype != torch.uint8 or state.numel() != batch * ny * nx or not state.is_contiguous()):
        raise ValueError("encode_fwd: `state` is the (B*ny*nx,) uint8 occupancy of the `out` canvases")
    lo = [float(torch.tensor(v, dtype=torch.float32)) for v in point_cloud_range[:3]]
    vs = [float(torch.tensor(v, dtype=torch.float32)) for v in voxel_size]
    if workspace.key[0] < batch or workspace.key[1] < n:
        raise ValueError("voxelize workspace too small for this call")
    check(lib().hvpr_encode_fwd_f32(
        _ptr(points, torch.float32, "points"), n, stride, xyz_col, n_feat, _ptr(frame_offsets, torch.int32, "frame_offsets"),
        batch, lo[0], lo[1], lo[2], vs[0], vs[1], vs[2], nx, ny, nz, int(max_points), int(max_voxels), int(cap_mode),
        float(offsets[0]), float(offsets[1]), float(offsets[2]),
        _ptr(folded["w0"], torch.float32), _ptr(folded["b0"], torch.float32), _ptr(folded["w1"], torch.float32),
        _ptr(folded["b1"], torch.float32), _ptr(folded["ws0"], torch.float32), _ptr(folded["bs0"], torch.float32),
        _ptr(folded["ws1"], torch.float32), _ptr(folded["bs1"], torch.float32), *_bank_args(bank), int(k), _ptr(voxels), coords.data_ptr(), num.data_ptr(), offs.data_ptr(), capacity, pf.data_ptr(),
        sf.data_ptr(), _ptr(mask), mem.data_ptr(), spatial.data_ptr(), spatial_scale.data_ptr(), _ptr(state), workspace.buf.data_ptr(),
        workspace.buf.numel(), workspace.key[0], workspace.key[1], int(index_mode), _stream()), "hvpr_encode_fwd_f32")
    return {"voxels": voxels, "coords": coords, "num_points": num, "voxel_offsets": offs, "pillar_features": pf,
            "pillar_scale_features": sf, "pillar_mask": mask, "memory_features": mem,
            "spatial": spatial.permute(0, 3, 1, 2), "spatial_scale": spatial_scale.permute(0, 3, 1, 2)}


def canvas_buffers(batch, nx, ny, device):
    sp = torch.zeros((batch, ny, nx, 128), dtype=torch.float32, device=device).permute(0, 3, 1, 2)
    sc = torch.zeros((batch, ny, nx, 32), dtype=torch.float32, device=device).permute(0, 3, 1, 2)
    return (sp, sc), torch.zeros((batch * ny * nx,), dtype=torch.uint8, device=device)


class PackedConv:

    __slots__ = ("w", "bias", "taps", "stride", "cout", "cout_pad", "up", "cin", "relu", "tile_cfg")

    def __init__(self, w, bias, taps, stride, cout, cout_pad, up, cin, relu, tile_cfg):
        self.w, self.bias, self.taps, self.stride = w, bias, taps, stride
        self.cout, self.cout_pad, self.up, self.cin, self.relu, self.tile_cfg = cout, cout_pad, up, cin, relu, tile_cfg


def _tile_channels(tile_cfg):
    return 128 if tile_cfg == 0 else 64


def pack_conv(weight, scale=None, shift=None, stride=1, relu=True, tile_cfg=0):
    cout, cin, kh, kw = weight.shape
    assert kh == kw and kh in (1, 3) and cin % 8 == 0
    w = weight.detach().float()
    if scale is not None:
        w = w * scale.view(-1, 1, 1, 1)
    tc = _tile_channels(tile_cfg)
    cout_pad = (cout + tc - 1) // tc * tc
    taps = kh * kw
    p = w.permute(2, 3, 1, 0).reshape(taps, cin // 8, 2, 4, cout).permute(0, 1, 2, 4, 3)
    wp = torch.zeros((taps, cin // 8, 2, cout_pad, 4), dtype=torch.float32, device=w.device)
    wp[:, :, :, :cout] = p
    b = torch.zeros((cout_pad,), dtype=torch.float32, device=w.device)
    if shift is not None:
        b[:cout] = shift.detach().float()
    return PackedConv(wp.contiguous(), b, taps, stride, cout, cout_pad, 1, cin, relu, tile_cfg)


_zero_bias = {}


class PackedConvWino:

    __slots__ = ("w", "bias", "cout", "cout_pad", "cin", "relu", "px_groups")
    taps, stride, up = 9, 1, 1

    def __init__(self, w, bias, cout, cout_pad, cin, relu, px_groups):
        self.w, self.bias, self.cout, self.cout_pad, self.cin, self.relu, self.px_groups = w, bias, cout, cout_pad, cin, relu, px_groups


def pack_conv_wino(weight, scale=None, shift=None, relu=True, px_groups=1, adjoint=False):
    w = weight.detach()
    if w.dtype != torch.float32 or not w.is_contiguous():
        w = w.float().contiguous()
    cout, cin = (w.shape[1], w.shape[0]) if adjoint else (w.shape[0], w.shape[1])
    assert w.shape[2:] == (3, 3) and cin % 8 == 0 and cout % 4 == 0
    cout_pad = (cout + 63) // 64 * 64
    wp = torch.empty((lib().hvpr_conv2d_wino_packed_floats(cin, cout),), dtype=torch.float32, device=w.device)
    sc = None if scale is None else scale.detach().float().contiguous()
    check(lib().hvpr_conv2d_wino_pack_f32(_ptr(w, torch.float32, "conv weight"), _ptr(sc, torch.float32, "scale"), cout, cin,
                                          1 if adjoint else 0, wp.data_ptr(), _stream()), "hvpr_conv2d_wino_pack_f32")
    if shift is None:
        key = (cout_pad, w.device)
        if key not in _zero_bias:
            _zero_bias[key] = torch.zeros((cout_pad,), dtype=torch.float32, device=w.device)
        b = _zero_bias[key]
    else:
        b = torch.zeros((cout_pad,), dtype=torch.float32, device=w.device)
        b[:cout] = shift.detach().float()
    return PackedConvWino(wp, b, cout, cout_pad, cin, relu, px_groups)


def conv2d_wino_nhwc(x, pc, out=None, out_coff=0, gate=None, resid=None, bn_partials=None):
    N, H, W, cin = x.shape
    assert cin == pc.cin
    if out is None:
        out = torch.empty((N, H, W, pc.cout), dtype=torch.float32, device=x.device)
    assert out.shape[:3] == (N, H, W) and out.is_contiguous()
    check(lib().hvpr_conv2d_wino_nhwc_f32(_ptr(x, torch.float32, "conv input"), N, H, W, cin, pc.w.data_ptr(), pc.bias.data_ptr(),
                                          pc.cout, 1 if pc.relu else 0, _ptr(gate, torch.float32, "gate"),
                                          _ptr(resid, torch.float32, "resid"), 0 if resid is None else resid.shape[-1],
                                          out.data_ptr(), out.shape[-1], int(out_coff), pc.px_groups,
                                          _ptr(bn_partials, torch.float32, "bn_partials"), _stream()), "hvpr_conv2d_wino_nhwc_f32")
    return out


def pack_deconv(weight, scale, shift, relu=True, tile_cfg=0):
    cin, cout, s, s2 = weight.shape
    assert s == s2 and cin % 8 == 0
    w = weight.detach().float() * scale.view(1, -1, 1, 1)
    cols = s * s * cout
    tc = _tile_channels(tile_cfg)
    cout_pad = (cols + tc - 1) // tc * tc
    g = w.permute(0, 2, 3, 1).reshape(cin, cols)
    p = g.reshape(cin // 8, 2, 4, cols).permute(0, 1, 3, 2).unsqueeze(0)
    wp = torch.zeros((1, cin // 8, 2, cout_pad, 4), dtype=torch.float32, device=w.device)
    wp[:, :, :, :cols] = p
    b = torch.zeros((cout_pad,), dtype=torch.float32, device=w.device)
    b[:cols] = shift.detach().float().repeat(s * s)
    return PackedConv(wp.contiguous(), b, 1, 1, cout, cout_pad, s, cin, relu, tile_cfg)


def conv_algo():
    algo = os.environ.get("HVPR_CONV_ALGO", "winograd")
    if algo not in ("winograd", "direct"):
        raise ValueError(f"HVPR_CONV_ALGO must be 'winograd' or 'direct', got {algo!r}")
    return algo


def pack_conv_auto(weight, scale=None, shift=None, stride=1, relu=True, tile_cfg=1, px_groups=1):
    if weight.shape[2] == 3 and stride == 1 and weight.shape[0] % 4 == 0 and weight.shape[1] % 8 == 0 and conv_algo() == "winograd":
        return pack_conv_wino(weight, scale, shift, relu=relu, px_groups=px_groups)
    return pack_conv(weight, scale, shift, stride=stride, relu=relu, tile_cfg=tile_cfg)


def conv2d_nhwc(x, pc, out=None, out_coff=0, gate=None, resid=None):
    if isinstance(pc, PackedConvBf3):
        if pc.up is not None:
            assert gate is None and resid is None
            return deconv_nhwc_bf3(x, pc, out, out_coff=out_coff)
        assert out is None, "the split-bf16 convolution allocates its own output"
        return conv2d_nhwc_bf3(x, pc, out_split=pc.out_split, gate=gate, resid=resid)
    if x.dtype == torch.bfloat16:
        x = unsplit_bf16(x)
    if isinstance(pc, PackedConvWino):
        return conv2d_wino_nhwc(x, pc, out=out, out_coff=out_coff, gate=gate, resid=resid)
    N, H, W, cin = x.shape
    assert cin == pc.cin
    if pc.taps == 9:
        OH, OW = (H + 2 - 3) // pc.stride + 1, (W + 2 - 3) // pc.stride + 1
    else:
        OH, OW = H, W
    if out is None:
        out = torch.empty((N, OH * pc.up, OW * pc.up, pc.cout), dtype=torch.float32, device=x.device)
    assert out.shape[:3] == (N, OH * pc.up, OW * pc.up) and out.is_contiguous()
    check(lib().hvpr_conv2d_nhwc_f32(_ptr(x, torch.float32, "conv input"), N, H, W, cin, pc.w.data_ptr(),
                                     pc.bias.data_ptr(), pc.taps, pc.stride, pc.cout, pc.cout_pad, pc.up,
                                     1 if pc.relu else 0, _ptr(gate, torch.float32, "gate"),
                                     _ptr(resid, torch.float32, "resid"), 0 if resid is None else resid.shape[-1],
                                     out.data_ptr(), out.shape[-1], int(out_coff), pc.tile_cfg, _stream()),
          "hvpr_conv2d_nhwc_f32")
    return out


def pack_conv_s2_dgrad(weight):
    return pack_conv(weight.detach().permute(1, 0, 2, 3), None, None, stride=1, relu=False, tile_cfg=1)


def conv2d_s2_dgrad_nhwc(dz, weight, H, W, pc=None):
    N, OH, OW, cout = dz.shape
    cin = weight.shape[1]
    assert weight.shape[0] == cout and tuple(weight.shape[2:]) == (3, 3) and OH == (H + 2 - 3) // 2 + 1 and OW == (W + 2 - 3) // 2 + 1
    if pc is None:
        pc = pack_conv_s2_dgrad(weight)
    dx = torch.empty((N, H, W, cin), dtype=torch.float32, device=dz.device)
    check(lib().hvpr_conv2d_s2_dgrad_nhwc_f32(_ptr(dz, torch.float32, "dz"), N, OH, OW, cout, pc.w.data_ptr(), pc.bias.data_ptr(), cin,
                                              pc.cout_pad, H, W, dx.data_ptr(), cin, 0, _stream()), "hvpr_conv2d_s2_dgrad_nhwc_f32")
    return dx


def spatial_gate(y_nhwc, w18, conv_bias, bn_scale, bn_shift):
    N, H, W, C = y_nhwc.shape
    gate = torch.empty((N, H, W), dtype=torch.float32, device=y_nhwc.device)
    check(lib().hvpr_spatial_gate_f32(_ptr(y_nhwc, torch.float32, "scale features"), N, H, W, C,
                                      _ptr(w18, torch.float32, "gate conv weight"), float(conv_bias), float(bn_scale),
                                      float(bn_shift), gate.data_ptr(), _stream()), "hvpr_spatial_gate_f32")
    return gate


def head_decode(head_nhwc, n_anchor, n_class, n_dir_bins, x_shifts, y_shifts, anchor_table, dir_offset, dir_limit_offset,
                period, want_cls=True, want_scores=True, out=None):
    N, H, W, CH = head_nhwc.shape
    A = H * W * n_anchor
    dev = head_nhwc.device
    if out is not None:
        cls, box, scores, labels = out
        if box.shape != (N, A, 7) or not all(t is None or t.is_contiguous() for t in out):
            raise ValueError("head_decode: `out` tensors do not match this call")
    else:
        cls = torch.empty((N, A, n_class), dtype=torch.float32, device=dev) if want_cls else None
        box = torch.empty((N, A, 7), dtype=torch.float32, device=dev)
        scores = torch.empty((N, A), dtype=torch.float32, device=dev) if want_scores else None
        labels = torch.empty((N, A), dtype=torch.int32, device=dev) if want_scores else None
    check(lib().hvpr_head_decode_f32(_ptr(head_nhwc, torch.float32, "head output"), N, H, W, CH, n_anchor, n_class,
                                     n_dir_bins, _ptr(x_shifts, torch.float32), _ptr(y_shifts, torch.float32),
                                     _ptr(anchor_table, torch.float32), float(dir_offset), float(dir_limit_offset),
                                     float(period), _ptr(cls), box.data_ptr(), _ptr(scores), _ptr(labels), _stream()),
          "hvpr_head_decode_f32")
    return cls, box, scores, labels


class PostWorkspace:

    def __init__(self, batch, n_scores, pre_max, device):
        self.batch, self.n_scores, self.pre_max = batch, n_scores, pre_max
        self.topk = torch.zeros(lib().hvpr_score_topk_workspace_bytes(batch, n_scores), dtype=torch.uint8, device=device)
        self.nms = torch.empty(lib().hvpr_nms_workspace_bytes(pre_max), dtype=torch.uint8, device=device)


def score_topk(scores, score_thresh, pre_max, ws, want_scores=True):
    B, A = scores.shape
    if B != ws.batch:
        raise ValueError(f"score_topk: {B} frames on a workspace made for {ws.batch}")
    dev = scores.device
    order = torch.empty((B, pre_max), dtype=torch.int32, device=dev)
    ss = torch.empty((B, pre_max), dtype=torch.float32, device=dev) if want_scores else None
    counts = torch.empty((B,), dtype=torch.int32, device=dev)
    use = score_thresh is not None
    check(lib().hvpr_score_topk_f32(_ptr(scores, torch.float32, "scores"), B, A, float(score_thresh) if use else 0.0,
                                    1 if use else 0, int(pre_max), order.data_ptr(), _ptr(ss), counts.data_ptr(),
                                    ws.topk.data_ptr(), ws.topk.numel(), _stream()), "hvpr_score_topk_f32")
    return order, ss, counts


def nms_bev(boxes, order, n_device, n_max, thresh, max_keep, ws_nms, map_through_order=True):
    dev = boxes.device
    keep = torch.zeros((max(max_keep, 1),), dtype=torch.int32, device=dev)
    kc = torch.empty((1,), dtype=torch.int32, device=dev)
    check(lib().hvpr_nms_bev_f32(_ptr(boxes, torch.float32, "boxes"), boxes.shape[1], _ptr(order, torch.int32),
                                 _ptr(n_device, torch.int32), int(n_max), float(thresh), int(max_keep),
                                 1 if map_through_order else 0, keep.data_ptr(), kc.data_ptr(), ws_nms.data_ptr(),
                                 ws_nms.numel(), _stream()), "hvpr_nms_bev_f32")
    return keep, kc


def gather_predictions(boxes, scores, labels, keep):
    K = keep.shape[0]
    dev = boxes.device
    ob = torch.empty((K, 7), dtype=torch.float32, device=dev)
    os_ = torch.empty((K,), dtype=torch.float32, device=dev)
    ol = torch.empty((K,), dtype=torch.int64, device=dev)
    osel = torch.empty((K,), dtype=torch.int64, device=dev)
    check(lib().hvpr_gather_predictions_f32(_ptr(boxes, torch.float32, "boxes"), boxes.shape[1], _ptr(scores, torch.float32, "scores"),
                                            _ptr(labels, torch.int32, "labels"), _ptr(keep, torch.int32, "keep"), K, ob.data_ptr(),
                                            os_.data_ptr(), ol.data_ptr(), osel.data_ptr(), _stream()), "hvpr_gather_predictions_f32")
    return ob, os_, ol, osel


def boxes_pairwise(a, b, mode):
    a = a[:, :7].contiguous()
    b = b[:, :7].contiguous()
    out = torch.zeros((a.shape[0], b.shape[0]), dtype=torch.float32, device=a.device)
    check(lib().hvpr_boxes_pairwise_f32(_ptr(a, torch.float32, "boxes_a"), a.shape[0], _ptr(b, torch.float32, "boxes_b"),
                                        b.shape[0], int(mode), out.data_ptr(), _stream()), "hvpr_boxes_pairwise_f32")
    return out
```

### hvpr_amd/map_to_bev.py

```python
import math

import torch
import torch.nn as nn

from . import kernels


class MemoryUnit_Agg(nn.Module):

    def __init__(self, mem_dim, fea_dim, shrink_thres=0.0025):
        super().__init__()
        self.mem_dim, self.fea_dim, self.shrink_thres = mem_dim, fea_dim, shrink_thres
        self.weight = nn.Parameter(torch.empty(mem_dim, fea_dim))
        stdv = 1.0 / math.sqrt(fea_dim)
        self.weight.data.uniform_(-stdv, stdv)
        self._packed = None

    def train(self, mode=True):
        self._packed = None
        return super().train(mode)

    def _load_from_state_dict(self, *a, **k):
        self._packed = None
        return super()._load_from_state_dict(*a, **k)

    def packed_bank(self):
        w = self.weight
        key = (w.data_ptr(), w._version, w.device)
        if self._packed is None or self._packed[0] != key:
            self._packed = (key, kernels.PackedBank(w) if (w.is_cuda and w.shape[1] == 64) else w.detach().contiguous())
        return self._packed[1]

    def forward(self, input1, k, input2=None):
        if self.training:
            return self._forward_train(input1, k, input2)
        return {"output": kernels.memory_readout_fwd(input1.contiguous(), self.packed_bank(), k)}

    def _check_train(self, t, d):
        if not t.is_cuda:
            raise RuntimeError("hvpr_amd: the memory training branch needs GPU tensors (the HIP path has no CPU fallback)")
        if d != 64 or self.mem_dim > 2048 or not self.shrink_thres > 0:
            raise ValueError("hvpr_amd: the memory training branch is built for 64 channels, <= 2048 items and SHRINK_TH > 0 (hvpr.yaml:83-85)")

    def _forward_train(self, pillars, k, positives):
        nv, _, d = positives.shape
        self._check_train(positives, d)
        mem = _MemoryTrain.apply(positives.reshape(-1, d), self.weight, float(self.shrink_thres))
        return {"output": _AttendRows.apply(pillars, mem, None, None)}

    def forward_train_indexed(self, pillars, k, points, idx, plan=None):
        nv, d = idx.shape[0], points.shape[1]
        self._check_train(points, d)
        mem_points = _MemoryTrain.apply(points, self.weight, float(self.shrink_thres))
        return {"output": _AttendRows.apply(pillars, mem_points, idx, plan)}

    def extra_repr(self):
        return f"mem_dim={self.mem_dim}, fea_dim={self.fea_dim}"


class _MemoryTrain(torch.autograd.Function):

    @staticmethod
    def _ws(n_items, device):
        return torch.empty(kernels.lib().hvpr_memory_train_workspace_bytes(n_items), dtype=torch.uint8, device=device)

    @staticmethod
    def forward(ctx, x, weight, lambd):
        x, w = x.contiguous(), weight.detach().contiguous()
        R, n_items = x.shape[0], w.shape[0]
        y = torch.empty_like(x)
        stats = torch.empty((R, 4), dtype=torch.float32, device=x.device)
        ws = _MemoryTrain._ws(n_items, x.device)
        kernels.check(kernels.lib().hvpr_memory_train_fwd_f32(kernels._ptr(x, torch.float32, "x"), R, kernels._ptr(w, torch.float32, "memory.weight"),
                                                              n_items, lambd, y.data_ptr(), stats.data_ptr(), ws.data_ptr(), ws.numel(),
                                                              kernels._stream()), "hvpr_memory_train_fwd_f32")
        ctx.save_for_backward(x, w, stats)
        ctx.lambd = lambd
        return y

    @staticmethod
    def backward(ctx, dy):
        x, w, stats = ctx.saved_tensors
        dy = dy.contiguous()
        R, n_items = x.shape[0], w.shape[0]
        dx, dw = torch.empty_like(x), torch.empty_like(w)
        scratch = torch.empty((2 * max(R, 1),), dtype=torch.float32, device=x.device)
        ws = _MemoryTrain._ws(n_items, x.device)
        kernels.check(kernels.lib().hvpr_memory_train_bwd_f32(x.data_ptr(), kernels._ptr(dy, torch.float32, "dy"), R, w.data_ptr(), n_items, ctx.lambd,
                                                              stats.data_ptr(), dx.data_ptr(), dw.data_ptr(), scratch.data_ptr(), ws.data_ptr(),
                                                              ws.numel(), kernels._stream()), "hvpr_memory_train_bwd_f32")
        return dx, dw, None


class _GatherRows(torch.autograd.Function):

    @staticmethod
    def forward(ctx, rows, idx, plan=None):
        rows = rows.contiguous()
        flat = idx.reshape(-1).to(torch.int32).contiguous()
        out = torch.empty((flat.numel(), rows.shape[1]), dtype=torch.float32, device=rows.device)
        kernels.check(kernels.lib().hvpr_gather_rows_f32(kernels._ptr(rows, torch.float32, "rows"), rows.shape[0], rows.shape[1], flat.data_ptr(),
                                                         flat.numel(), out.data_ptr(), kernels._stream()), "hvpr_gather_rows_f32")
        ctx.save_for_backward(flat)
        ctx.n = rows.shape[0]
        ctx.plan = plan
        return out.view(*idx.shape, rows.shape[1])

    @staticmethod
    def backward(ctx, grad):
        (flat,) = ctx.saved_tensors
        grad = grad.contiguous()
        c = grad.shape[-1]
        order, chunk_ptr, dest_ptr = ctx.plan.get() if ctx.plan is not None else kernels.edges_by_destination(flat.to(torch.int64), ctx.n)
        g = kernels.segment_sum_rows(grad.reshape(-1, c), 0, c, order, None, chunk_ptr, dest_ptr, ctx.n)
        return g, None, None


class _EdgePlan:

    def __init__(self, idx, n):
        self.idx, self.n, self._plan, self._owner, self._i32 = idx, n, None, None, None

    def get(self):
        if self._plan is None:
            self._plan = kernels.edges_by_destination(self.idx.reshape(-1).to(torch.int64), self.n)
        return self._plan

    def idx32(self):
        if self._i32 is None:
            self._i32 = self.idx.to(torch.int32).contiguous()
        return self._i32

    def owner(self):
        if self._owner is None:
            self._owner = torch.div(self.get()[0], self.idx.shape[-1], rounding_mode="floor")
        return self._owner


class _AttendRows(torch.autograd.Function):

    @staticmethod
    def forward(ctx, q, rows, idx, plan=None):
        q, rows = q.detach().contiguous(), rows.detach().contiguous()
        if idx is None:
            if rows.shape[0] % max(q.shape[0], 1):
                raise ValueError("hvpr_amd: the dense attend needs rows (M * k, C) for q (M, C)")
            out, w = kernels.attend_rows(q, rows, None, rows.shape[0] // q.shape[0] if q.shape[0] else 1)
        else:
            if plan is None:
                plan = _EdgePlan(idx, rows.shape[0])
            out, w = kernels.attend_rows(q, rows, plan.idx32())
        ctx.save_for_backward(w)
        ctx.plan, ctx.n = plan, rows.shape[0]
        return out

    @staticmethod
    def backward(ctx, grad):
        (w,) = ctx.saved_tensors
        if not ctx.needs_input_grad[1]:
            return None, None, None, None
        grad = grad.contiguous()
        if ctx.plan is None:
            return None, (w.unsqueeze(2) * grad.unsqueeze(1)).reshape(ctx.n, grad.shape[1]), None, None
        order, chunk_ptr, dest_ptr = ctx.plan.get()
        edge_w = torch.index_select(w.reshape(-1), 0, order)
        g = kernels.segment_sum_rows(grad, 0, grad.shape[1], ctx.plan.owner(), edge_w, chunk_ptr, dest_ptr, ctx.n)
        return None, g, None, None


class _ScatterCanvas(torch.autograd.Function):

    @staticmethod
    def forward(ctx, feats, coords_i32, batch, nx, ny, ws):
        c = feats.shape[1]
        if c == 128:
            sp, _ = kernels.scatter_bev_fwd(feats[:, :64].contiguous(), feats[:, 64:].contiguous(), None, coords_i32, batch, nx, ny, ws)
        elif c == 64:
            sp, _ = kernels.scatter_bev_fwd(feats.contiguous(), None, None, coords_i32, batch, nx, ny, ws)
        else:
            assert c < 64
            pad = torch.cat([feats, feats.new_zeros(feats.shape[0], 64 - c)], dim=1)
            sp = kernels.scatter_bev_fwd(pad, None, None, coords_i32, batch, nx, ny, ws)[0][:, :c]
        rows = ((coords_i32[:, 0] * ny + coords_i32[:, 2]) * nx + coords_i32[:, 3]).contiguous()
        ctx.save_for_backward(rows)
        ctx.c = c
        return sp

    @staticmethod
    def backward(ctx, grad):
        (rows,) = ctx.saved_tensors
        g = grad.permute(0, 2, 3, 1).contiguous()
        cells, ch = g.shape[0] * g.shape[1] * g.shape[2], g.shape[3]
        out = torch.empty((rows.shape[0], ch), dtype=torch.float32, device=g.device)
        kernels.check(kernels.lib().hvpr_gather_rows_f32(kernels._ptr(g, torch.float32, "grad canvas"), cells, ch, rows.data_ptr(), rows.shape[0],
                                                         out.data_ptr(), kernels._stream()), "hvpr_gather_rows_f32")
        return (out if ch == ctx.c else out[:, :ctx.c].contiguous()), None, None, None, None, None


class _ScatterBase(nn.Module):
    def __init__(self, model_cfg, grid_size, **kwargs):
        super().__init__()
        self.model_cfg = model_cfg
        self.num_bev_features = model_cfg.NUM_BEV_FEATURES
        self.nx, self.ny, self.nz = [int(g) for g in grid_size]
        assert self.nz == 1
        self._ws = None

    def _workspace(self, batch, device):
        if self._ws is None or self._ws[0] != (batch, device):
            self._ws = ((batch, device), kernels.scatter_workspace(batch, self.nx, self.ny, device))
        return self._ws[1]


def _coords_i32(batch_dict):
    c = batch_dict["voxel_coords"]
    return (c if c.dtype == torch.int32 else c.to(torch.int32)).contiguous()


def _batch_size(batch_dict):
    if "batch_size" in batch_dict:
        return int(batch_dict["batch_size"])
    return int(batch_dict["voxel_coords"][:, 0].max().item()) + 1


class PointPillarScatter(_ScatterBase):

    def forward(self, batch_dict, **kwargs):
        pf = batch_dict["pillar_features"]
        B = _batch_size(batch_dict)
        sp, _ = kernels.scatter_bev_fwd(pf.contiguous(), None, None, _coords_i32(batch_dict), B, self.nx, self.ny,
                                        self._workspace(B, pf.device), m_device=batch_dict.get("voxel_count_device"))
        batch_dict["spatial_features"] = sp
        return batch_dict


def _frame_ranges(cols, B):
    parts = []
    for c in cols:
        c = c.long()
        ok = ((c[1:] >= c[:-1]).sum() == max(c.numel() - 1, 0)) & ((c >= 0) & (c < B)).sum().eq(c.numel())
        cnt = (c.view(-1, 1) == torch.arange(B, device=c.device).view(1, -1)).sum(dim=0)
        parts += [cnt, ok.view(1).long()]
    host = torch.cat(parts).tolist()
    out = []
    for i in range(len(cols)):
        cnt, ok = host[i * (B + 1):i * (B + 1) + B], host[i * (B + 1) + B]
        if not ok:
            out.append(None)
            continue
        lo, r = 0, []
        for n in cnt:
            r.append((lo, lo + n))
            lo += n
        out.append(r)
    return out


class PointPillarScatter_Agg_Memory_1_scale(_ScatterBase):

    def __init__(self, model_cfg, grid_size, **kwargs):
        super().__init__(model_cfg, grid_size)
        self.num_coord_points = model_cfg.NUM_COORD_POINTS
        self.num_pt_features = model_cfg.NUM_PT_FEATURES
        self.num_scale_features = model_cfg.NUM_SCALE_FEATURES
        self.k = model_cfg.NUM_K
        self.mem_size = model_cfg.NUM_M
        self.shrink_thres = model_cfg.SHRINK_TH
        self.memory = MemoryUnit_Agg(self.mem_size, self.num_pt_features, self.shrink_thres)

    def get_score(self, points, pillars):
        with torch.no_grad():
            idx = self._topk_points(pillars.detach(), points.detach())
        positives = _GatherRows.apply(points, idx)
        return _AttendRows.apply(pillars, positives.reshape(-1, positives.shape[2]), None, None), positives

    def _topk_points(self, pillars, points):
        k, N = self.k, points.shape[0]
        nb = 1
        if not pillars.is_cuda:
            raise RuntimeError("hvpr_amd: get_score needs GPU tensors (the HIP path has no CPU fallback)")
        if pillars.shape[1] != 64:
            raise ValueError("hvpr_amd: get_score is built for 64-channel point / pillar features (hvpr.yaml:81)")
        if pillars.shape[0] == 0:
            return torch.zeros((0, k), dtype=torch.long, device=pillars.device)
        if N < k * max(nb, 1):
            raise ValueError(f"hvpr_amd: get_score needs at least k = {k} points per sample, got {N}")
        pf, pts = pillars.contiguous(), points.contiguous()
        packed = kernels.PackedBank(pts)
        idx = torch.empty((pf.shape[0], k), dtype=torch.int32, device=pf.device)
        kernels.check(kernels.lib().hvpr_point_pillar_topk_f32(kernels._ptr(pf, torch.float32, "pillars"), pf.shape[0], packed.rows.data_ptr(),
                                                               packed.data.data_ptr(), N, k, idx.data_ptr(), kernels._stream()),
                      "hvpr_point_pillar_topk_f32")
        return idx.long()

    def _forward_train(self, batch_dict):
        pf, sf = batch_dict["pillar_features"], batch_dict["pillar_scale_features"]
        coords = _coords_i32(batch_dict)
        point_f, point_c = batch_dict["point_features"], batch_dict["point_coords"]
        B = _batch_size(batch_dict)
        pos_point, pos_mem = [], []
        vr, pr = _frame_ranges([coords[:, 0], point_c[:, 0]], B)
        if vr is not None and pr is not None:
            with torch.no_grad():
                picks = [self._topk_points(pf[v0:v1].detach(), point_f[p0:p1].detach()) + p0
                         for (v0, v1), (p0, p1) in zip(vr, pr) if v1 > v0]
            idx = torch.cat(picks, 0) if picks else torch.zeros((0, self.k), dtype=torch.long, device=pf.device)
            plan = _EdgePlan(idx, point_f.shape[0])
            pos_point = _AttendRows.apply(pf, point_f, idx, plan)
            pos_mem = self.memory.forward_train_indexed(pf, self.k, point_f, idx, plan)["output"]
        else:
            for b in range(B):
                agg, positives = self.get_score(point_f[point_c[:, 0] == b], pf[coords[:, 0] == b])
                pos_point.append(agg)
                pos_mem.append(self.memory(pf[coords[:, 0] == b], self.k, positives)["output"])
            pos_point, pos_mem = torch.cat(pos_point, 0), torch.cat(pos_mem, 0)
        ws = self._workspace(B, pf.device)
        args = (coords, B, self.nx, self.ny, ws)
        batch_dict["spatial_features"] = _ScatterCanvas.apply(torch.cat([pf.detach(), pos_mem], dim=1), *args)
        batch_dict["spatial_features_point"] = _ScatterCanvas.apply(torch.cat([pf, pos_point], dim=1), *args)
        batch_dict["spatial_scale_features"] = _ScatterCanvas.apply(sf, *args)
        batch_dict["point_positive_features"] = pos_point
        batch_dict["memory_positive_features"] = pos_mem
        batch_dict["memory_items"] = self.memory.weight
        return batch_dict

    def forward(self, batch_dict, **kwargs):
        if self.training:
            return self._forward_train(batch_dict)
        pf, sf = batch_dict["pillar_features"], batch_dict["pillar_scale_features"]
        md = batch_dict.get("voxel_count_device")
        B = _batch_size(batch_dict)
        bank = self.memory.packed_bank()
        if pf.shape[1] == 64 and sf.shape[1] == 32 and bank.shape[1] == 64:
            _, sp, sc = kernels.memory_scatter_fwd(pf.contiguous(), sf.contiguous(), _coords_i32(batch_dict), bank, self.k, B,
                                                   self.nx, self.ny, self._workspace(B, pf.device), m_device=md,
                                                   out=batch_dict.get("_out_spatial"))
        else:
            mem = kernels.memory_readout_fwd(pf.contiguous(), bank, self.k, m_device=md)
            sp, sc = kernels.scatter_bev_fwd(pf.contiguous(), mem, sf.contiguous(), _coords_i32(batch_dict), B, self.nx,
                                             self.ny, self._workspace(B, pf.device), m_device=md)
        batch_dict["spatial_features"] = sp
        batch_dict["spatial_scale_features"] = sc
        return batch_dict


__all__ = {
    "PointPillarScatter": PointPillarScatter,
    "PointPillarScatter_Agg_Memory_1_scale": PointPillarScatter_Agg_Memory_1_scale,
}
```

### include/hvpr_amd.h

```cpp
#ifndef HVPR_AMD_H
#define HVPR_AMD_H

#include <stddef.h>
#include <stdint.h>

#ifdef __cplusplus
extern "C" {
#endif

typedef void *hvpr_stream_t;

enum hvpr_status {
    HVPR_OK = 0,
    HVPR_ERR_INVALID_ARG = -1,
    HVPR_ERR_UNSUPPORTED = -2,
    HVPR_ERR_WORKSPACE = -3,
    HVPR_ERR_LAUNCH = -4,
    HVPR_ERR_TIMEOUT = -5
};

int hvpr_abi_version(void);
const char *hvpr_status_string(int status);

typedef int (*hvpr_allreduce_fn)(double *buf, int n, hvpr_stream_t stream, void *ctx);
void hvpr_set_batchnorm_allreduce(hvpr_allreduce_fn fn, void *ctx);

size_t hvpr_voxelize_workspace_bytes(int max_batch, int max_points, int nx, int ny, int nz);
int hvpr_voxelize_workspace_reset(void *workspace, size_t workspace_bytes, int max_batch, int max_points, int nx, int ny,
                                  int nz, hvpr_stream_t stream);
int hvpr_voxelize_workspace_status(const void *workspace, size_t workspace_bytes, int max_batch, int max_points, int nx, int ny,
                                   int nz, hvpr_stream_t stream);
int hvpr_voxelize_f32(const float *points, int n_points, int point_stride, int xyz_col, int n_feat,
                      const int32_t *frame_offsets, int batch, float lo_x, float lo_y, float lo_z, float vs_x,
                      float vs_y, float vs_z, int nx, int ny, int nz, int max_points, int max_voxels, int cap_mode,
                      float *voxels, int32_t *coords, int32_t *num_points, int32_t *voxel_offsets, int capacity,
                      void *workspace, size_t workspace_bytes, int ws_max_batch, int ws_max_points,
                      hvpr_stream_t stream);

int hvpr_pillar_vfe_fwd_f32(const float *voxels, const int32_t *num_points, const int32_t *coords, int M, int P,
                            const int32_t *m_device, float vs_x, float vs_y, float vs_z, float off_x, float off_y,
                            float off_z, const float *w0, const float *b0, const float *w1, const float *b1,
                            const float *ws0, const float *bs0, const float *ws1, const float *bs1,
                            float *pillar_features, float *pillar_scale_features, float *pillar_mask,
                            hvpr_stream_t stream);

size_t hvpr_pillar_vfe_train_workspace_bytes(void);
int hvpr_pillar_vfe_train_fwd_f32(const float *voxels, const int32_t *num_points, const int32_t *coords, int M, int P, const float *w0,
                                  const float *gamma0, const float *beta0, const float *w1, const float *gamma1, const float *beta1,
                                  float eps, float vs_x, float vs_y, float vs_z, float off_x, float off_y, float off_z,
                                  float *pillar_features, float *mean0, float *var0, float *mean1, float *var1, void *workspace,
                                  size_t workspace_bytes, hvpr_stream_t stream);
int hvpr_pillar_vfe_bwd_f32(const float *voxels, const int32_t *num_points, const int32_t *coords, int M, int P, const float *w0,
                            const float *gamma0, const float *beta0, const float *w1, const float *gamma1, const float *beta1, float eps,
                            float vs_x, float vs_y, float vs_z, float off_x, float off_y, float off_z, const float *d_pillar_features,
                            float *dw0, float *dgamma0, float *dbeta0, float *dw1, float *dgamma1, float *dbeta1, void *workspace,
                            size_t workspace_bytes, hvpr_stream_t stream);

size_t hvpr_memory_bank_packed_floats(int n_items);
int hvpr_memory_bank_pack_f32(const float *bank, int n_items, float *packed, hvpr_stream_t stream);
int hvpr_memory_readout_fwd_f32(const float *f, int M, const int32_t *m_device, const float *bank, const float *bank_packed,
                                int n_items, int k, float *out, int32_t *topk_idx, hvpr_stream_t stream);

size_t hvpr_scatter_workspace_bytes(int batch, int nx, int ny);
int hvpr_scatter_bev_fwd_f32(const float *pillar_features, int c_pillar, const float *memory_features, int c_mem,
                             const float *scale_features, int c_scale, const int32_t *coords, int M,
                             const int32_t *m_device, int batch, int nx, int ny, float *spatial,
                             float *spatial_scale, void *workspace, size_t workspace_bytes, hvpr_stream_t stream);

int hvpr_memory_scatter_fwd_f32(const float *pillar_features, const float *scale_features, const int32_t *coords, int M,
                                const int32_t *m_device, const float *bank, const float *bank_packed, int n_items, int k, int batch,
                                int nx, int ny,
                                float *memory_features, float *spatial, float *spatial_scale, void *workspace,
                                size_t workspace_bytes, hvpr_stream_t stream);

int hvpr_encode_fwd_f32(const float *points, int n_points, int point_stride, int xyz_col, int n_feat,
                        const int32_t *frame_offsets, int batch, float lo_x, float lo_y, float lo_z, float vs_x, float vs_y,
                        float vs_z, int nx, int ny, int nz, int max_points, int max_voxels, int cap_mode, float off_x,
                        float off_y, float off_z, const float *w0, const float *b0, const float *w1, const float *b1,
                        const float *ws0, const float *bs0, const float *ws1, const float *bs1, const float *bank,
                        const float *bank_packed, int n_items, int k, float *voxels, int32_t *coords, int32_t *num_points, int32_t *voxel_offsets,
                        int capacity, float *pillar_features, float *pillar_scale_features, float *pillar_mask,
                        float *memory_features, float *spatial, float *spatial_scale, uint8_t *canvas_state, void *workspace,
                        size_t workspace_bytes, int ws_max_batch, int ws_max_points, int index_mode, hvpr_stream_t stream);

int hvpr_conv2d_nhwc_f32(const float *in, int N, int H, int W, int Cin, const float *w_packed, const float *bias,
                         int taps, int stride, int cout, int cout_pad, int up, int relu, const float *gate,
                         const float *resid, int resid_cstride, float *out, int out_cstride, int out_coff,
                         int tile_cfg, hvpr_stream_t stream);

int hvpr_spatial_gate_f32(const float *y, int N, int H, int W, int C, const float *w18, float conv_bias, float bn_scale,
                          float bn_shift, float *gate, hvpr_stream_t stream);

int hvpr_head_decode_f32(const float *head, int N, int H, int W, int head_channels, int n_anchor, int n_class,
                         int n_dir_bins, const float *x_shifts, const float *y_shifts, const float *anchor_table,
                         float dir_offset, float dir_limit_offset, float period, float *batch_cls_preds,
                         float *batch_box_preds, float *scores, int32_t *labels, hvpr_stream_t stream);

size_t hvpr_score_topk_workspace_bytes(int batch, int n_scores);
int hvpr_score_topk_f32(const float *scores, int batch, int n_scores, float score_thresh, int use_thresh, int pre_max,
                        int32_t *order, float *sorted_scores, int32_t *counts, void *workspace, size_t workspace_bytes,
                        hvpr_stream_t stream);

size_t hvpr_nms_workspace_bytes(int n_max);
int hvpr_nms_bev_f32(const float *boxes, int box_stride, const int32_t *order, const int32_t *n_device, int n_max,
                     float thresh, int max_keep, int map_through_order, int32_t *keep, int32_t *keep_count,
                     void *workspace, size_t workspace_bytes, hvpr_stream_t stream);
int hvpr_gather_predictions_f32(const float *boxes, int box_stride, const float *scores, const int32_t *labels,
                                const int32_t *keep, int max_keep, float *out_boxes, float *out_scores, int64_t *out_labels,
                                int64_t *out_selected, hvpr_stream_t stream);
int hvpr_boxes_pairwise_f32(const float *boxes_a, int n, const float *boxes_b, int m, int mode, float *out,
                            hvpr_stream_t stream);

int hvpr_furthest_point_sample_f32(const float *xyz, int B, int N, int npoint, int32_t *idx, hvpr_stream_t stream);
int hvpr_ball_query_f32(const float *xyz, const float *new_xyz, int B, int N, int M, float radius, int nsample, int32_t *idx,
                        hvpr_stream_t stream);
int hvpr_three_nn_f32(const float *unknown, const float *known, int B, int n, int m, float *dist, int32_t *idx,
                      hvpr_stream_t stream);

int hvpr_group_points_f32(const float *features, const int32_t *idx, int B, int C, int N, int npoint, int nsample, float *out,
                          hvpr_stream_t stream);
int hvpr_group_points_grad_f32(const float *grad_out, const int32_t *idx, int B, int C, int N, int npoint, int nsample,
                               float *grad_features, hvpr_stream_t stream);
int hvpr_three_interpolate_f32(const float *features, const int32_t *idx, const float *weight, int B, int C, int m, int n,
                               float *out, hvpr_stream_t stream);
int hvpr_three_interpolate_grad_f32(const float *grad_out, const int32_t *idx, const float *weight, int B, int C, int m, int n,
                                    float *grad_features, hvpr_stream_t stream);
int hvpr_group_rows_f32(const float *xyz, const float *features, const float *new_xyz, const int32_t *idx, int B, int N, int C,
                        int npoint, int nsample, int cpad, float *out, hvpr_stream_t stream);
int hvpr_max_samples_f32(const float *y, long long G, int nsample, int C, float *out, uint8_t *argmax, hvpr_stream_t stream);
int hvpr_max_samples_grad_f32(const float *grad_out, const uint8_t *argmax, long long G, int nsample, int C, float *grad_y,
                              hvpr_stream_t stream);
int hvpr_fp_rows_f32(const float *known, const int32_t *idx, const float *weight, const float *skip, int B, int m, int n, int C1,
                     int C2, int cpad, float *out, hvpr_stream_t stream);
size_t hvpr_spatial_gate_train_workspace_bytes(int N, int H, int W);
int hvpr_spatial_gate_train_fwd_f32(const float *y, int N, int H, int W, int C, const float *w18, const float *conv_bias,
                                    const float *gamma, const float *beta, float eps, float *pooled, int32_t *argmax, float *a,
                                    float *stats, float *gate, void *workspace, size_t workspace_bytes, hvpr_stream_t stream);
int hvpr_spatial_gate_train_bwd_f32(const float *dgate, const float *gate, const float *a, const float *stats, const float *pooled,
                                    const int32_t *argmax, const float *w18, const float *gamma, int N, int H, int W, int C,
                                    float *dy, float *dw18, float *dbias, float *dgamma, float *dbeta, void *workspace,
                                    size_t workspace_bytes, hvpr_stream_t stream);
int hvpr_point_pillar_topk_f32(const float *pillars, int M, const float *points, const float *points_packed, int N, int k,
                               int32_t *idx, hvpr_stream_t stream);
int hvpr_scatter_add_rows_f32(const float *src, const int32_t *idx, long long m, int row_floats, int n_dst, float *dst,
                              hvpr_stream_t stream);

int hvpr_segment_sum_rows_f32(const float *src, long long src_stride, int src_off, int C, const int32_t *edge_row,
                              const float *edge_w, const int32_t *rowptr, long long n_dst, float *dst, long long dst_stride,
                              hvpr_stream_t stream);

int hvpr_attend_rows_fwd_f32(const float *q, int M, const float *rows, long long N, const int32_t *idx, int k, int C, float *out,
                             float *w, hvpr_stream_t stream);

size_t hvpr_memory_train_workspace_bytes(int n_items);
int hvpr_memory_train_fwd_f32(const float *x, long long R, const float *bank, int n_items, float shrink_thres, float *y, float *row_stats,
                              void *workspace, size_t workspace_bytes, hvpr_stream_t stream);
int hvpr_memory_train_bwd_f32(const float *x, const float *dy, long long R, const float *bank, int n_items, float shrink_thres,
                              const float *row_stats, float *dx, float *dbank, float *row_scratch, void *workspace,
                              size_t workspace_bytes, hvpr_stream_t stream);

size_t hvpr_conv2d_wino_wgrad_workspace_bytes(int N, int H, int W, int Cin, int Cout);
int hvpr_conv2d_wino_wgrad_nhwc_f32(const float *x, int N, int H, int W, int Cin, const float *dz, int Cout, float *dw,
                                    void *workspace, size_t workspace_bytes, hvpr_stream_t stream);
size_t hvpr_conv2d_wgrad_workspace_bytes(int N, int OH, int OW, int Cin, int Cout, int taps, int stride);
int hvpr_conv2d_wgrad_nhwc_f32(const float *x, int N, int H, int W, int Cin, const float *dz, int Cout, int taps, int stride, float *dw,
                               void *workspace, size_t workspace_bytes, hvpr_stream_t stream);
int hvpr_conv2d_s2_dgrad_nhwc_f32(const float *dz, int N, int H, int W, int Cin, const float *w_packed, const float *bias, int cout,
                                  int cout_pad, int OH, int OW, float *dx, int out_cstride, int out_coff, hvpr_stream_t stream);

size_t hvpr_bn_workspace_bytes(long long P, int C);
int hvpr_bn_stats_nhwc_f32(const float *z, long long P, int C, float eps, float *mean, float *var, float *invstd, void *workspace,
                           size_t workspace_bytes, hvpr_stream_t stream);
int hvpr_bn_finalize_partials_f32(const float *partials, int rows, int C, long long count, float eps, float *mean, float *var,
                                  float *invstd, hvpr_stream_t stream);
int hvpr_bn_train_affine_f32(const float *mean, const float *var, const float *invstd, int C, const float *gamma, const float *beta,
                             float momentum, float momentum_unbiased, float *running_mean, float *running_var,
                             long long *num_batches_tracked, float *scale, float *shift, hvpr_stream_t stream);
int hvpr_bn_relu_fwd_nhwc_f32(const float *z, long long P, int C, const float *scale, const float *shift, int relu, const float *gate,
                              const float *resid, float *y, int y_cstride, int y_coff, hvpr_stream_t stream);
int hvpr_bn_relu_bwd_sums_nhwc_f32(const float *dy, int dy_cstride, int dy_coff, const float *z, long long P, int C, const float *scale,
                                   const float *shift, const float *mean, const float *invstd, int relu, const float *gate, float *dgamma,
                                   float *dbeta, void *workspace, size_t workspace_bytes, hvpr_stream_t stream);
int hvpr_bn_relu_bwd_apply_nhwc_f32(const float *dy, int dy_cstride, int dy_coff, const float *z, long long P, int C, const float *scale,
                                    const float *shift, const float *mean, const float *invstd, int relu, const float *gate, float *dgate,
                                    float *dz, const float *dgamma_total, const float *dbeta_total, double inv_count, hvpr_stream_t stream);

size_t hvpr_assign_targets_workspace_bytes(int batch, int n_gt);
int hvpr_assign_targets_f32(const float *anchors, int n_anchors, const float *gt_boxes, int batch, int n_gt, int class_index,
                            int n_classes, float matched_thr, float unmatched_thr, int per_loc, int loc_stride, int loc_offset,
                            long long anchors_total, int32_t *labels, float *reg_targets, float *reg_weights, int32_t *pos_count,
                            void *workspace, size_t workspace_bytes, hvpr_stream_t stream);

size_t hvpr_rpn_losses_workspace_bytes(int batch, long long n_anchors);
int hvpr_rpn_losses_f32(const float *cls_preds, const float *box_preds, const float *dir_preds, const int32_t *labels,
                        const float *reg_targets, const float *anchor_rot, const int32_t *pos_count, int batch, long long n_anchors,
                        int num_class, int num_dir_bins, float alpha, float gamma, float beta, const float *code_weights,
                        float cls_weight, float loc_weight, float dir_weight, float dir_offset, float *losses, float *grad_cls,
                        float *grad_box, float *grad_dir, void *workspace, size_t workspace_bytes, hvpr_stream_t stream);
size_t hvpr_mse_loss_workspace_bytes(void);
int hvpr_mse_loss_f32(const float *x, const float *target, long long rows, int cols, float weight, float *loss, float *grad_x,
                      void *workspace, size_t workspace_bytes, hvpr_stream_t stream);

int hvpr_fused_adam_truewd_f32(float *params, const float *grads, float *exp_avg, float *exp_avg_sq, long long n, float lr,
                               float beta1, float beta2, float eps, float weight_decay, int step,
                               const float *grad_scale_device, hvpr_stream_t stream);


size_t hvpr_conv2d_wino_packed_floats(int cin, int cout);
int hvpr_conv2d_wino_pack_f32(const float *weight, const float *scale, int cout, int cin, int adjoint, float *packed,
                              hvpr_stream_t stream);
int hvpr_conv2d_wino_nhwc_f32(const float *in, int N, int H, int W, int Cin, const float *w_packed, const float *bias, int cout,
                              int relu, const float *gate, const float *resid, int resid_cstride, float *out, int out_cstride,
                              int out_coff, int px_groups, float *bn_partials, hvpr_stream_t stream);
int hvpr_conv2d_wino_stats_rows(int N, int H, int W);

int hvpr_split_bf16_f32(const float *src, long long n_floats, int n_planes, void *dst, hvpr_stream_t stream);
int hvpr_unsplit_bf16_f32(const void *src, long long n_floats, int n_planes, float *dst, hvpr_stream_t stream);
int hvpr_conv2d_nhwc_bf16x3(const void *in_split, int N, int H, int W, int Cin, const void *w_split, const float *bias,
                            int stride, int cout, int cout_pad, int relu, const float *gate, const void *resid_split,
                            int resid_cstride, void *out, int out_split, int out_cstride, int out_coff, int tile_cfg,
                            int n_planes, hvpr_stream_t stream);
int hvpr_deconv_nhwc_bf16x3(const void *in_split, int N, int H, int W, int Cin, const void *w_split, const float *bias, int cout,
                            int cout_pad, int up, int relu, float *out, int out_cstride, int out_coff, int n_planes,
                            hvpr_stream_t stream);

int hvpr_point_flags_f32(const float *points, int n, int stride, int mode, const float *range_xy, float near_thresh,
                         const float *fov_lidar_to_rect, const float *fov_rect_to_img, int img_h, int img_w, uint8_t *flags,
                         hvpr_stream_t stream);
size_t hvpr_compact_workspace_bytes(int n);
int hvpr_compact_rows_f32(const float *src, int n, int row_floats, const uint8_t *flags, float *dst, int capacity,
                          int32_t *count, void *workspace, size_t workspace_bytes, hvpr_stream_t stream);
int hvpr_gather_rows_f32(const float *src, int n_src, int row_floats, const int32_t *idx, int m, float *dst,
                         hvpr_stream_t stream);
int hvpr_frame_offsets_f32(const float *points, int n_points, int point_stride, int batch, int32_t *frame_offsets,
                           hvpr_stream_t stream);

#ifdef __cplusplus
}
#endif
#endif
```

Measured before the change: 455.0 frames/s.

## Skip Winograd conv work on empty BEV tiles using a per-frame occupancy tile plan

Adds a GPU kernel that builds, from the pillar coordinates, a per-tile distance-to-nearest-occupied key and a sorted tile order. The level-0 Winograd convolutions then compute only tiles within the receptive-field reach of occupied pillars at each depth. Remaining tiles are filled with a precomputed 2x2-periodic background pattern, obtained at plan build time by running the layers on an all-zero canvas. This targets the mostly empty KITTI BEV canvas, at the cost of an extra planning kernel and a correctness dependence on the background periodicity check and the border handling.

```diff
diff --git a/hvpr_amd/_lib.py b/hvpr_amd/_lib.py
--- a/hvpr_amd/_lib.py
+++ b/hvpr_amd/_lib.py
@@ -94,6 +94,9 @@
     "hvpr_conv2d_wino_pack_f32": (_I, [_P, _P, _I, _I, _I, _P, _P]),
     "hvpr_conv2d_wino_nhwc_f32": (_I, [_P, _I, _I, _I, _I, _P, _P, _I, _I, _P, _P, _I, _P, _I, _I, _I, _P, _P]),
     "hvpr_conv2d_wino_stats_rows": (_I, [_I, _I, _I]),
+    "hvpr_bev_tile_plan_bytes": (_Z, [_I, _I, _I]),
+    "hvpr_bev_tile_plan": (_I, [_P, _P, _I, _I, _I, _I, _P, _P]),
+    "hvpr_conv2d_wino_tiled_nhwc_f32": (_I, [_P, _I, _I, _I, _I, _P, _P, _I, _I, _P, _P, _I, _P, _I, _I, _P, _I, _P, _P]),
     "hvpr_conv2d_s2_dgrad_nhwc_f32": (_I, [_P, _I, _I, _I, _I, _P, _P, _I, _I, _I, _I, _P, _I, _I, _P]),
     "hvpr_bn_train_affine_f32": (_I, [_P, _P, _P, _I, _P, _P, _F, _F, _P, _P, _P, _P, _P, _P]),
     "hvpr_bn_finalize_partials_f32": (_I, [_P, _I, _I, _c.c_longlong, _F, _P, _P, _P, _P]),
diff --git a/hvpr_amd/bev_backbone.py b/hvpr_amd/bev_backbone.py
--- a/hvpr_amd/bev_backbone.py
+++ b/hvpr_amd/bev_backbone.py
@@ -1,6 +1,7 @@
 import collections
 import contextlib
 import os
+import warnings
 
 import torch
 import torch.nn as nn
@@ -41,7 +42,7 @@
 _WINO_PX_GROUPS = 1
 
 _Level = collections.namedtuple("_Level", "index trunk scale gate sfm_steps deconv coff")
-_Plan = collections.namedtuple("_Plan", "levels planes")
+_Plan = collections.namedtuple("_Plan", "levels planes bg")
 
 
 def _fold_pack(pack, conv, bn, **kw):
@@ -94,19 +95,23 @@
         self.held.clear()
 
 
-def _trunk(lv, x, out=None):
-    for pc in lv.trunk[:-1]:
-        x = kernels.conv2d_nhwc(x, pc)
-    return kernels.conv2d_nhwc(x, lv.trunk[-1], out=out)
-
-
-def _branch(lv, x, y, out, fork, y_out=None):
+def _tiles(sparse, depth):
+    return None if sparse is None else (sparse[0], depth, sparse[1][depth - 1])
+
+
+def _trunk(lv, x, out=None, sparse=None):
+    for d, pc in enumerate(lv.trunk):
+        x = kernels.conv2d_nhwc(x, pc, out=out if d == len(lv.trunk) - 1 else None, tiles=_tiles(sparse, d + 1))
+    return x
+
+
+def _branch(lv, x, y, out, fork, y_out=None, sparse=None):
     with fork.branch(lv.index, x, out):
         y = kernels.conv2d_nhwc(y, lv.scale, out=y_out)
         fork.y_ready(lv.index, y)
         gate = kernels.spatial_gate(y, *lv.gate)
-        for pc in lv.sfm_steps:
-            x = kernels.conv2d_nhwc(x, pc, gate=gate, resid=x)
+        for d, pc in enumerate(lv.sfm_steps):
+            x = kernels.conv2d_nhwc(x, pc, gate=gate, resid=x, tiles=_tiles(sparse, len(lv.trunk) + d + 1))
             fork.held.append(x)
         fork.held.append(gate)
         kernels.conv2d_nhwc(x, lv.deconv, out=out, out_coff=lv.coff)
@@ -202,7 +207,33 @@
                 sfm_steps[-1] = sfm.fp32_output()
             levels.append(_Level(i, trunk, scale, gate, sfm_steps, deconv, coff))
             coff += self.up_filters[i]
-        return _Plan(levels, planes)
+        return _Plan(levels, planes, self._background_blocks(levels[0]) if not planes else None)
+
+    def _background_blocks(self, lv):
+        layers = list(lv.trunk) + list(lv.sfm_steps)
+        if self.layer_strides[0] != 1 or len(layers) > 9 or not isinstance(lv.scale, kernels.PackedConvWino) or \
+                not all(isinstance(pc, kernels.PackedConvWino) and pc.px_groups == 1 for pc in layers):
+            return None
+        dev = layers[0].w.device
+        H, W = 40, 48
+        x = torch.zeros((1, H, W, layers[0].cin), dtype=torch.float32, device=dev)
+        y = torch.zeros((1, H, W, lv.scale.cin), dtype=torch.float32, device=dev)
+        outs = []
+        for pc in lv.trunk:
+            x = kernels.conv2d_nhwc(x, pc)
+            outs.append(x)
+        gate = kernels.spatial_gate(kernels.conv2d_nhwc(y, lv.scale), *lv.gate)
+        for pc in lv.sfm_steps:
+            x = kernels.conv2d_nhwc(x, pc, gate=gate, resid=x)
+            outs.append(x)
+        bg = []
+        for o in outs:
+            tile, blk = o[0, 16:24, 16:32], o[0, 16:18, 16:18].contiguous()
+            if not torch.equal(tile, blk.repeat(4, 8, 1)):
+                warnings.warn("hvpr_amd: a level-0 layer is not 2x2-periodic on an empty canvas; the empty-field skip is off")
+                return None
+            bg.append(blk)
+        return bg
 
     def _forward_train(self, data_dict):
         if not data_dict["spatial_features"].is_cuda:
@@ -255,12 +286,17 @@
         data_dict["spatial_features_point_2d"] = ct.bn_relu_cat(ups_p, bns).permute(0, 3, 1, 2)
         return data_dict
 
-    def _head(self, plan, x, y, out, level, x_out={}, y_out=None):
+    def _head(self, plan, x, y, out, level, x_out={}, y_out=None, tile_plan=None):
         fork = _Fork(self._streams(y.device))
+        sparse = None
+        if tile_plan is not None and plan.bg is not None and kernels.bev_sparse_enabled():
+            assert tile_plan.numel() == kernels.bev_tile_plan_ints(*x.shape[:3]), "the tile plan belongs to another canvas"
+            sparse = (tile_plan, plan.bg)
         for lv in plan.levels:
-            x = _trunk(lv, x, out=x_out.get(lv.index))
+            first = lv.index == 0
+            x = _trunk(lv, x, out=x_out.get(lv.index), sparse=sparse if first else None)
             if lv.index < level:
-                y = _branch(lv, x, y, out, fork, y_out=y_out if lv.index == level - 1 else None)
+                y = _branch(lv, x, y, out, fork, y_out=y_out if lv.index == level - 1 else None, sparse=sparse if first else None)
         fork.join()
 
     def forward(self, data_dict):
@@ -274,15 +310,15 @@
                           dtype=torch.float32, device=x.device)
         if plan.planes:
             x = kernels.split_bf16(x, plan.planes)
-        self._head(plan, x, y, out, len(plan.levels))
+        self._head(plan, x, y, out, len(plan.levels), tile_plan=data_dict.get("bev_tile_plan"))
         data_dict["spatial_features_2d"] = out.permute(0, 3, 1, 2)
         return data_dict
 
-    def forward_head(self, spatial, scale, split):
+    def forward_head(self, spatial, scale, split, tile_plan=None):
         y = _nhwc(scale)
         plan = self._fold.get(y.device, self._build_plan)
         assert not plan.planes, "the split forward runs the fp32 kernels"
-        self._head(plan, _nhwc(spatial), y, split["out"], split["level"], split["x"], split["y"])
+        self._head(plan, _nhwc(spatial), y, split["out"], split["level"], split["x"], split["y"], tile_plan=tile_plan)
 
     def forward_tail(self, split):
         y, out = split["y"], split["out"]
diff --git a/hvpr_amd/csrc/bev_tile_plan.hip b/hvpr_amd/csrc/bev_tile_plan.hip
--- /dev/null
+++ b/hvpr_amd/csrc/bev_tile_plan.hip
@@ -0,0 +1,114 @@
+#include "internal.h"
+
+namespace {
+
+constexpr int PT = 1024, NW = PT / 64;
+constexpr int KEY_CAP = 9, NKEY = KEY_CAP + 1;
+constexpr int TH = 8, TW = 16;
+constexpr int LDS_TILES = 8192;
+constexpr int TICKET = 11;
+
+__global__ void __launch_bounds__(PT) k_tile_plan(const int4 *__restrict__ coords, const int *__restrict__ count_dev, int m_rows, int N,
+                                                  int H, int W, int tiles_y, int tiles_x, int *__restrict__ plan) {
+    __shared__ int s_key[LDS_TILES];
+    __shared__ int s_hist[NKEY], s_base[NKEY], s_wave[NW][NKEY];
+    __shared__ int s_last;
+    const int tid = threadIdx.x, lane = tid & 63, wid = tid >> 6;
+    const int n_tiles = N * tiles_y * tiles_x;
+    int *const order = plan + kTilePlanHeader;
+    int *const key_g = order + n_tiles;
+    int *const near = key_g + n_tiles;
+
+    int live = m_rows;
+    if (count_dev) live = min(max(*count_dev, 0), m_rows);
+    for (int p = blockIdx.x * PT + tid; p < live; p += gridDim.x * PT) {
+        const int4 c = coords[p];
+        const int b = c.x, y = c.z, x = c.w;
+        if (b < 0 || b >= N || y < 0 || y >= H || x < 0 || x >= W) continue;
+        const int ty_lo = max(y - (KEY_CAP - 1), 0) / TH, ty_hi = min(y + (KEY_CAP - 1), H - 1) / TH;
+        const int tx_lo = max(x - (KEY_CAP - 1), 0) / TW, tx_hi = min(x + (KEY_CAP - 1), W - 1) / TW;
+        for (int ty = ty_lo; ty <= ty_hi; ++ty)
+            for (int tx = tx_lo; tx <= tx_hi; ++tx) {
+                const int y0 = ty * TH, y1 = min(y0 + TH, H) - 1, x0 = tx * TW, x1 = min(x0 + TW, W) - 1;
+                const int d = max(max(max(y0 - y, y - y1), max(x0 - x, x - x1)), 0);
+                int *const w = &near[(b * tiles_y + ty) * tiles_x + tx];
+                if (d < KEY_CAP && __hip_atomic_load(w, __ATOMIC_RELAXED, __HIP_MEMORY_SCOPE_AGENT) < KEY_CAP - d) atomicMax(w, KEY_CAP - d);
+            }
+    }
+    __threadfence();
+    __syncthreads();
+    if (tid == 0) s_last = atomicAdd(&plan[TICKET], 1) == (int)gridDim.x - 1;
+    __syncthreads();
+    if (!s_last) return;
+    __threadfence();
+
+    int *const key = n_tiles <= LDS_TILES ? s_key : key_g;
+    if (tid < NKEY) s_hist[tid] = 0;
+    __syncthreads();
+    for (int t = tid; t < n_tiles; t += PT) {
+        const int tx = t % tiles_x, ty = (t / tiles_x) % tiles_y;
+        const int y0 = ty * TH, y1 = min(y0 + TH, H) - 1, x0 = tx * TW, x1 = min(x0 + TW, W) - 1;
+        const int bd = min(min(y0, x0), min(H - 1 - y1, W - 1 - x1));
+        const int nr = min(max(atomicExch(&near[t], 0), 0), KEY_CAP);
+        const int k = min(KEY_CAP - nr, bd + 2);
+        key[t] = k;
+        if (key != key_g) key_g[t] = k;
+        atomicAdd(&s_hist[k], 1);
+    }
+    if (tid == 0) atomicExch(&plan[TICKET], 0);
+    __syncthreads();
+    if (tid == 0) {
+        int run = 0;
+        for (int k = 0; k < NKEY; ++k) {
+            s_base[k] = run;
+            run += s_hist[k];
+            plan[k] = run;
+        }
+        plan[NKEY] = n_tiles;
+    }
+    __syncthreads();
+    for (int t0 = 0; t0 < n_tiles; t0 += PT) {
+        const int t = t0 + tid;
+        const int k = t < n_tiles ? key[t] : -1;
+        int rank = 0;
+#pragma unroll
+        for (int q = 0; q < NKEY; ++q) {
+            const unsigned long long m = __ballot(k == q);
+            if (lane == 0) s_wave[wid][q] = __popcll(m);
+            if (k == q) rank = __popcll(m & ((1ull << lane) - 1ull));
+        }
+        __syncthreads();
+        if (k >= 0) {
+            int pos = s_base[k] + rank;
+            for (int w = 0; w < wid; ++w) pos += s_wave[w][k];
+            order[pos] = t;
+        }
+        __syncthreads();
+        if (tid < NKEY) {
+            int add = 0;
+            for (int w = 0; w < NW; ++w) add += s_wave[w][tid];
+            s_base[tid] += add;
+        }
+        __syncthreads();
+    }
+}
+
+}
+
+extern "C" size_t hvpr_bev_tile_plan_bytes(int N, int H, int W) {
+    if (N < 1 || H < 1 || W < 1) return 0;
+    const size_t tiles = (size_t)N * ((H + TH - 1) / TH) * ((W + TW - 1) / TW);
+    return (kTilePlanHeader + 3 * tiles) * sizeof(int);
+}
+
+extern "C" int hvpr_bev_tile_plan(const int32_t *voxel_coords, const int32_t *voxel_count, int m_rows, int N, int H, int W, int32_t *plan,
+                                  hvpr_stream_t stream) {
+    if (!plan || N < 1 || H < 1 || W < 1 || m_rows < 0 || (m_rows > 0 && !voxel_coords)) return HVPR_ERR_INVALID_ARG;
+    const int tiles_y = (H + TH - 1) / TH, tiles_x = (W + TW - 1) / TW;
+    if ((long long)N * tiles_y * tiles_x > (1ll << 24)) return HVPR_ERR_UNSUPPORTED;
+    const int blocks = m_rows > 256 * PT ? 256 : (m_rows > PT ? (m_rows + PT - 1) / PT : 1);
+    hipLaunchKernelGGL(k_tile_plan, dim3(blocks), dim3(PT), 0, (hipStream_t)stream, (const int4 *)voxel_coords, voxel_count, m_rows, N, H, W,
+                       tiles_y, tiles_x, plan);
+    HVPR_CHECK_LAUNCH();
+    return HVPR_OK;
+}
diff --git a/hvpr_amd/csrc/conv_wino.hip b/hvpr_amd/csrc/conv_wino.hip
--- a/hvpr_amd/csrc/conv_wino.hip
+++ b/hvpr_amd/csrc/conv_wino.hip
@@ -1,6 +1,6 @@
 #include <type_traits>
 
-#include "common.h"
+#include "internal.h"
 
 namespace {
 
@@ -36,6 +36,9 @@
     int relu;
     int tiles_x, tiles_y, n_ct;
     float *stats;
+    const int *plan;
+    const float *bg;
+    int depth;
 };
 
 __device__ __forceinline__ float4 f4_fma(float s, float4 a, float4 b) {
@@ -44,7 +47,7 @@
 __device__ __forceinline__ float4 f4_add(float4 a, float4 b) { return make_float4(a.x + b.x, a.y + b.y, a.z + b.z, a.w + b.w); }
 __device__ __forceinline__ float4 f4_sub(float4 a, float4 b) { return make_float4(a.x - b.x, a.y - b.y, a.z - b.z, a.w - b.w); }
 
-template <int NG, bool STATS, int NB>
+template <int NG, bool STATS, int NB, bool TILED = false>
 __global__ void __launch_bounds__(256 * NG) __attribute__((amdgpu_waves_per_eu(2, NB == 2 ? 2 : 3))) k_wino(WinoArgs a) {
     constexpr int NT = 256 * NG;
     constexpr int TH = 8 * NG, PH = TH + 2;
@@ -84,13 +87,19 @@
     const unsigned lds_patch0 = lds_addr_of(s_patch) + wave_s * 1024u;
 
     const int n_pt = a.tiles_x * a.tiles_y * a.N;
-    const int total_walk = ((n_pt + 7) / 8) * 8 * a.n_ct;
+    static_assert(!TILED || (NG == 1 && !STATS), "the tile plan is made of 8 x 16 pixel tiles");
+    const int n_act = TILED ? min(max(a.plan[a.depth], 0), n_pt) : n_pt;
+    const int total_walk = ((n_act + 7) / 8) * 8 * a.n_ct;
     const int n_chunks = a.Cin / KC;
     for (int it = blockIdx.x; it < total_walk; it += gridDim.x) {
     const int xcd = it & 7, j = it >> 3;
     const int ct = j % a.n_ct;
     int pt = (j / a.n_ct) * 8 + xcd;
-    if (pt >= n_pt) continue;
+    if (pt >= n_act) continue;
+    if (TILED) {
+        pt = a.plan[kTilePlanHeader + pt];
+        if ((unsigned)pt >= (unsigned)n_pt) continue;
+    }
     const int tx = pt % a.tiles_x; pt /= a.tiles_x;
     const int ty = pt % a.tiles_y;
     const int n = pt / a.tiles_y;
@@ -279,6 +288,23 @@
     }
     __syncthreads();
     }
+    if (TILED) {
+        const int n_fill = n_pt - n_act, c4 = a.cout >> 2;
+        const float4 *bg4 = (const float4 *)a.bg;
+        for (int fi = (int)(gridDim.x - 1 - blockIdx.x); fi < n_fill; fi += gridDim.x) {
+            int pt = a.plan[kTilePlanHeader + n_act + fi];
+            if ((unsigned)pt >= (unsigned)n_pt) continue;
+            const int tx = pt % a.tiles_x; pt /= a.tiles_x;
+            const int ty = pt % a.tiles_y;
+            const int n = pt / a.tiles_y;
+            for (int e = tid; e < TH * TW * c4; e += NT) {
+                const int c = e % c4, px = e / c4;
+                const int oy = ty * TH + px / TW, ox = tx * TW + px % TW;
+                if (oy < a.H && ox < a.W)
+                    *(float4 *)(a.out + (((size_t)n * a.H + oy) * a.W + ox) * a.out_cstride + a.out_coff + 4 * c) = bg4[((oy & 1) * 2 + (ox & 1)) * c4 + c];
+            }
+        }
+    }
 }
 
 __global__ void k_wino_pack(const float *__restrict__ w, const float *__restrict__ scale, int cout, int cin, int cout_pad, int adjoint,
@@ -313,7 +339,7 @@
     }
 }
 
-template <int NG, bool STATS, int NB>
+template <int NG, bool STATS, int NB, bool TILED = false>
 int launch(WinoArgs a, hipStream_t s) {
     constexpr int NT = 256 * NG, TH = 8 * NG, PH = TH + 2;
     constexpr int PPAD = (PH * ROWP + 63) / 64 * 64;
@@ -323,19 +349,19 @@
     a.tiles_y = (a.H + TH - 1) / TH;
     a.n_ct = a.cout_pad / (32 * NB);
     static unsigned long long lds_set = 0ull;
-    if (hvpr_ensure_dyn_lds((const void *)k_wino<NG, STATS, NB>, lds, &lds_set) != 0) return -1;
+    if (hvpr_ensure_dyn_lds((const void *)k_wino<NG, STATS, NB, TILED>, lds, &lds_set) != 0) return -1;
     const long long tiles = (long long)a.N * a.tiles_x * a.tiles_y * a.n_ct;
     static int resident = 0;
     if (resident == 0) {
         int per_cu = 0, dev = 0, cus = 256;
         hipDeviceProp_t prop;
         if (hipGetDevice(&dev) == hipSuccess && hipGetDeviceProperties(&prop, dev) == hipSuccess) cus = prop.multiProcessorCount;
-        if (hipOccupancyMaxActiveBlocksPerMultiprocessor(&per_cu, k_wino<NG, STATS, NB>, NT, lds) != hipSuccess || per_cu < 1) per_cu = 1;
+        if (hipOccupancyMaxActiveBlocksPerMultiprocessor(&per_cu, k_wino<NG, STATS, NB, TILED>, NT, lds) != hipSuccess || per_cu < 1) per_cu = 1;
         resident = per_cu * cus;
     }
     long long blocks = tiles < resident ? (tiles + 7) / 8 * 8 : resident;
     if (blocks > resident && resident >= 8) blocks = resident / 8 * 8;
-    hipLaunchKernelGGL((k_wino<NG, STATS, NB>), dim3((unsigned)blocks), dim3(NT), lds, s, a);
+    hipLaunchKernelGGL((k_wino<NG, STATS, NB, TILED>), dim3((unsigned)blocks), dim3(NT), lds, s, a);
     return 0;
 }
 
@@ -378,6 +404,7 @@
     a.out_cstride = out_cstride; a.out_coff = out_coff; a.resid_cstride = resid_cstride;
     a.relu = relu;
     a.stats = bn_partials;
+    a.plan = nullptr; a.bg = nullptr; a.depth = 0;
     if (bn_partials && (px_groups != 1 || relu || gate)) return HVPR_ERR_UNSUPPORTED;
     int rc;
     if (px_groups == 1) rc = bn_partials ? launch<1, true, 2>(a, (hipStream_t)stream) : launch<1, false, 2>(a, (hipStream_t)stream);
@@ -388,3 +415,29 @@
     HVPR_CHECK_LAUNCH();
     return HVPR_OK;
 }
+
+extern "C" int hvpr_conv2d_wino_tiled_nhwc_f32(const float *in, int N, int H, int W, int Cin, const float *w_packed, const float *bias,
+                                               int cout, int relu, const float *gate, const float *resid, int resid_cstride, float *out,
+                                               int out_cstride, int out_coff, const int32_t *plan, int depth, const float *background,
+                                               hvpr_stream_t stream) {
+    if (!plan)
+        return hvpr_conv2d_wino_nhwc_f32(in, N, H, W, Cin, w_packed, bias, cout, relu, gate, resid, resid_cstride, out, out_cstride, out_coff,
+                                         1, nullptr, stream);
+    if (!in || !w_packed || !bias || !out || !background || N < 1 || H < 1 || W < 1 || Cin < 8 || cout < 1) return HVPR_ERR_INVALID_ARG;
+    if (depth < 1 || depth > 9) return HVPR_ERR_INVALID_ARG;
+    if ((gate == nullptr) != (resid == nullptr)) return HVPR_ERR_INVALID_ARG;
+    if (Cin % KC != 0) return HVPR_ERR_UNSUPPORTED;
+    if (cout % 4 != 0 || out_cstride % 4 != 0 || out_coff % 4 != 0 || (resid && resid_cstride % 4 != 0)) return HVPR_ERR_UNSUPPORTED;
+    if ((long long)H * W * Cin * 4 >= (1ll << 31)) return HVPR_ERR_UNSUPPORTED;
+    WinoArgs a;
+    a.in = in; a.wpk = w_packed; a.bias = bias; a.out = out; a.gate = gate; a.resid = resid;
+    a.N = N; a.H = H; a.W = W; a.Cin = Cin;
+    a.cout = cout; a.cout_pad = (cout + BN - 1) / BN * BN;
+    a.out_cstride = out_cstride; a.out_coff = out_coff; a.resid_cstride = resid_cstride;
+    a.relu = relu;
+    a.stats = nullptr;
+    a.plan = plan; a.bg = background; a.depth = depth;
+    if (launch<1, false, 2, true>(a, (hipStream_t)stream) != 0) return HVPR_ERR_LAUNCH;
+    HVPR_CHECK_LAUNCH();
+    return HVPR_OK;
+}
diff --git a/hvpr_amd/csrc/internal.h b/hvpr_amd/csrc/internal.h
--- a/hvpr_amd/csrc/internal.h
+++ b/hvpr_amd/csrc/internal.h
@@ -7,6 +7,7 @@
 constexpr int kScanItems = 2;
 constexpr int kScanTile = kScanThreads * kScanItems;
 constexpr int kIdle = 0x7fffffff;
+constexpr int kTilePlanHeader = 16;
 
 struct VoxWs {
     int *cell_first;
diff --git a/hvpr_amd/detector.py b/hvpr_amd/detector.py
--- a/hvpr_amd/detector.py
+++ b/hvpr_amd/detector.py
@@ -344,14 +344,21 @@
                           voxel_count_device=vo[B:B + 1], pillar_features=r["pillar_features"],
                           pillar_scale_features=r["pillar_scale_features"], pillar_mask=r["pillar_mask"],
                           spatial_features=r["spatial"], spatial_scale_features=r["spatial_scale"])
+        if kernels.bev_sparse_enabled():
+            buf = batch_dict.get("_out_tile_plan")
+            if buf is None:
+                buf = kernels.bev_tile_plan_buffer(B, m.ny, m.nx, pts.device)
+            batch_dict["bev_tile_plan"] = kernels.bev_tile_plan(r["coords"], vo[B:B + 1], B, m.ny, m.nx, out=buf)
         return batch_dict
 
     def persistent_canvases(self, example_batch):
         if not self._can_fuse_encode(example_batch):
             return {}
         m = self.map_to_bev_module
-        canv, state = kernels.canvas_buffers(example_batch["batch_size"], m.nx, m.ny, example_batch["points"].device)
-        return {"_out_spatial": canv, "_canvas_state": state}
+        B, dev = example_batch["batch_size"], example_batch["points"].device
+        canv, state = kernels.canvas_buffers(B, m.nx, m.ny, dev)
+        plan = torch.zeros((kernels.bev_tile_plan_ints(B, m.ny, m.nx),), dtype=torch.int32, device=dev)
+        return {"_out_spatial": canv, "_canvas_state": state, "_out_tile_plan": plan}
 
     def stage_encode(self, batch_dict):
         if self._can_fuse_encode(batch_dict):
@@ -364,7 +371,8 @@
         return self.dense_head(self.backbone_2d(batch_dict))
 
     def stage_dense_a(self, batch_dict, split):
-        self.backbone_2d.forward_head(batch_dict["spatial_features"], batch_dict["spatial_scale_features"], split)
+        self.backbone_2d.forward_head(batch_dict["spatial_features"], batch_dict["spatial_scale_features"], split,
+                                      tile_plan=batch_dict.get("bev_tile_plan"))
 
     def stage_dense_b(self, batch_dict, split):
         return self.dense_head({**batch_dict, "spatial_features_2d": self.backbone_2d.forward_tail(split)})
@@ -479,7 +487,7 @@
         self.B = example_batch["batch_size"]
         self.inp = [{k: (v.clone() if torch.is_tensor(v) else v) for k, v in example_batch.items()} for _ in range(2)]
         self.canvas, self.head, self.aux, self.split = [None, None], [None, None], [None, None], [None, None]
-        self.enc, self.f2d = [None, None], [None, None]
+        self.enc, self.f2d, self.plan = [None, None], [None, None], [None, None]
         self.own = [model.persistent_canvases(example_batch) if hasattr(model, "persistent_canvases") else {} for _ in range(2)]
         side = torch.cuda.Stream()
         side.wait_stream(torch.cuda.current_stream())
@@ -488,6 +496,7 @@
                 for _ in range(warmup):
                     bd = model.stage_encode({**self.inp[p], **self.own[p]})
                     self.canvas[p] = (bd["spatial_features"], bd["spatial_scale_features"])
+                    self.plan[p] = bd.get("bev_tile_plan") if bd.get("bev_tile_plan") is self.own[p].get("_out_tile_plan") else None
                     if depth == 4:
                         if self.split[p] is None:
                             sp = bd["spatial_features"]
@@ -518,6 +527,8 @@
                     self.enc[p] = {k: bd[k] for k in ("voxel_coords", "voxel_num_points", "voxel_offsets", "pillar_features",
                                                       "pillar_scale_features") if bd.get(k) is not None}
                 dense_in = {"batch_size": self.B, "spatial_features": self.canvas[q][0], "spatial_scale_features": self.canvas[q][1]}
+                if self.plan[q] is not None:
+                    dense_in["bev_tile_plan"] = self.plan[q]
                 if depth == 3:
                     self.f2d[q] = model.stage_dense({**dense_in, "_out_head": self.head[q]})["spatial_features_2d"]
                 else:
diff --git a/hvpr_amd/kernels.py b/hvpr_amd/kernels.py
--- a/hvpr_amd/kernels.py
+++ b/hvpr_amd/kernels.py
@@ -1,3 +1,4 @@
+import functools
 import os
 
 import torch
@@ -438,12 +439,53 @@
     return PackedConvWino(wp, b, cout, cout_pad, cin, relu, px_groups)
 
 
-def conv2d_wino_nhwc(x, pc, out=None, out_coff=0, gate=None, resid=None, bn_partials=None):
+def bev_sparse_enabled():
+    return os.environ.get("HVPR_BEV_SPARSE", "1") != "0"
+
+
+@functools.lru_cache(maxsize=None)
+def bev_tile_plan_ints(batch, H, W):
+    return lib().hvpr_bev_tile_plan_bytes(int(batch), int(H), int(W)) // 4
+
+
+_tile_plan_bufs = {}
+
+
+def bev_tile_plan_buffer(batch, H, W, device):
+    key = (int(batch), int(H), int(W), torch.device(device))
+    buf = _tile_plan_bufs.get(key)
+    if buf is None:
+        buf = _tile_plan_bufs[key] = torch.zeros((bev_tile_plan_ints(*key[:3]),), dtype=torch.int32, device=device)
+    return buf
+
+
+def bev_tile_plan(coords, voxel_count, batch, H, W, out=None):
+    n = bev_tile_plan_ints(int(batch), int(H), int(W))
+    if out is None:
+        out = torch.zeros((n,), dtype=torch.int32, device=coords.device)
+    assert out.dtype == torch.int32 and out.numel() == n and out.is_contiguous()
+    assert coords.dim() == 2 and coords.shape[1] == 4
+    check(lib().hvpr_bev_tile_plan(_ptr(coords, torch.int32, "voxel coords"), _ptr(voxel_count, torch.int32, "voxel count"),
+                                   coords.shape[0], int(batch), int(H), int(W), out.data_ptr(), _stream()), "hvpr_bev_tile_plan")
+    return out
+
+
+def conv2d_wino_nhwc(x, pc, out=None, out_coff=0, gate=None, resid=None, bn_partials=None, tiles=None):
     N, H, W, cin = x.shape
     assert cin == pc.cin
     if out is None:
         out = torch.empty((N, H, W, pc.cout), dtype=torch.float32, device=x.device)
     assert out.shape[:3] == (N, H, W) and out.is_contiguous()
+    if tiles is not None:
+        plan, depth, bg = tiles
+        assert bn_partials is None and pc.px_groups == 1 and bg.shape == (2, 2, pc.cout)
+        check(lib().hvpr_conv2d_wino_tiled_nhwc_f32(_ptr(x, torch.float32, "conv input"), N, H, W, cin, pc.w.data_ptr(), pc.bias.data_ptr(),
+                                                    pc.cout, 1 if pc.relu else 0, _ptr(gate, torch.float32, "gate"),
+                                                    _ptr(resid, torch.float32, "resid"), 0 if resid is None else resid.shape[-1],
+                                                    out.data_ptr(), out.shape[-1], int(out_coff), _ptr(plan, torch.int32, "tile plan"),
+                                                    int(depth), _ptr(bg, torch.float32, "background"), _stream()),
+              "hvpr_conv2d_wino_tiled_nhwc_f32")
+        return out
     check(lib().hvpr_conv2d_wino_nhwc_f32(_ptr(x, torch.float32, "conv input"), N, H, W, cin, pc.w.data_ptr(), pc.bias.data_ptr(),
                                           pc.cout, 1 if pc.relu else 0, _ptr(gate, torch.float32, "gate"),
                                           _ptr(resid, torch.float32, "resid"), 0 if resid is None else resid.shape[-1],
@@ -481,7 +523,7 @@
     return pack_conv(weight, scale, shift, stride=stride, relu=relu, tile_cfg=tile_cfg)
 
 
-def conv2d_nhwc(x, pc, out=None, out_coff=0, gate=None, resid=None):
+def conv2d_nhwc(x, pc, out=None, out_coff=0, gate=None, resid=None, tiles=None):
     if isinstance(pc, PackedConvBf3):
         if pc.up is not None:
             assert gate is None and resid is None
@@ -491,7 +533,8 @@
     if x.dtype == torch.bfloat16:
         x = unsplit_bf16(x)
     if isinstance(pc, PackedConvWino):
-        return conv2d_wino_nhwc(x, pc, out=out, out_coff=out_coff, gate=gate, resid=resid)
+        return conv2d_wino_nhwc(x, pc, out=out, out_coff=out_coff, gate=gate, resid=resid, tiles=tiles)
+    assert tiles is None, "the tile plan belongs to the Winograd kernel"
     N, H, W, cin = x.shape
     assert cin == pc.cin
     if pc.taps == 9:
diff --git a/hvpr_amd/map_to_bev.py b/hvpr_amd/map_to_bev.py
--- a/hvpr_amd/map_to_bev.py
+++ b/hvpr_amd/map_to_bev.py
@@ -341,6 +341,11 @@
                                              self.ny, self._workspace(B, pf.device), m_device=md)
         batch_dict["spatial_features"] = sp
         batch_dict["spatial_scale_features"] = sc
+        if kernels.bev_sparse_enabled():
+            buf = batch_dict.get("_out_tile_plan")
+            if buf is None:
+                buf = kernels.bev_tile_plan_buffer(B, self.ny, self.nx, pf.device)
+            batch_dict["bev_tile_plan"] = kernels.bev_tile_plan(_coords_i32(batch_dict), md, B, self.ny, self.nx, out=buf)
         return batch_dict
 
 
diff --git a/include/hvpr_amd.h b/include/hvpr_amd.h
--- a/include/hvpr_amd.h
+++ b/include/hvpr_amd.h
@@ -214,6 +214,13 @@
                               int out_coff, int px_groups, float *bn_partials, hvpr_stream_t stream);
 int hvpr_conv2d_wino_stats_rows(int N, int H, int W);
 
+size_t hvpr_bev_tile_plan_bytes(int N, int H, int W);
+int hvpr_bev_tile_plan(const int32_t *voxel_coords, const int32_t *voxel_count, int m_rows, int N, int H, int W, int32_t *plan,
+                       hvpr_stream_t stream);
+int hvpr_conv2d_wino_tiled_nhwc_f32(const float *in, int N, int H, int W, int Cin, const float *w_packed, const float *bias, int cout,
+                                    int relu, const float *gate, const float *resid, int resid_cstride, float *out, int out_cstride,
+                                    int out_coff, const int32_t *plan, int depth, const float *background, hvpr_stream_t stream);
+
 int hvpr_split_bf16_f32(const float *src, long long n_floats, int n_planes, void *dst, hvpr_stream_t stream);
 int hvpr_unsplit_bf16_f32(const void *src, long long n_floats, int n_planes, float *dst, hvpr_stream_t stream);
 int hvpr_conv2d_nhwc_bf16x3(const void *in_split, int N, int H, int W, int Cin, const void *w_split, const float *bias,
```

Measured after the change: 498.0 frames/s (median of 6 runs). 1.09x the previous value.
